# JiehongLin/SAM-6D

Hardware: NVIDIA H100
Metric: poses/sec (higher is better)
Workload: dtype bf16

## Files before the change

include/sam6d_b200.h:

```cpp
#ifndef SAM6D_B200_H
#define SAM6D_B200_H

#ifdef __cplusplus
extern "C" {
#endif


int sam6d_fps(const float* xyz, int b, int n, int m, float* temp, int* idx, void* stream);
int sam6d_fps_single_cta(const float* xyz, int b, int n, int m, float* temp, int* idx, void* stream);

int sam6d_gather_points(const float* points, const int* idx, int b, int c, int n, int m, float* out, void* stream);

int sam6d_gather_rows(const float* src, const int* idx, int b, int n, int m, int c, long long src_bstride, float* out,
                      void* stream);
int sam6d_gather_rows_bf16_f32(const void* src, const int* idx, int b, int n, int m, int c, long long src_bstride, float* out,
                               void* stream);

int sam6d_ball_query(const float* new_xyz, const float* xyz, int b, int n, int m, float radius, int nsample, int* idx,
                     int* cnt, void* stream);
int sam6d_ball_query_pair(const float* new_xyz, const float* xyz, int b, int n, int m, float radius_a, int nsample_a,
                          float radius_b, int nsample_b, int* idx_a, int* idx_b, int* cnt_a, int* cnt_b, void* stream);

int sam6d_group_points(const float* points, const int* idx, int b, int c, int n, int np, int ns, float* out, void* stream);


int sam6d_gemm_f32(const float* A, const float* W, const float* bias, const float* R, float* C, int M, int N, int K,
                   long long lda, long long ldw, long long ldc, long long ldr, int batch, long long sA, long long sW,
                   long long sC, long long sR, float alpha, int relu, void* stream);

int sam6d_gemm_bf16(const void* A, int a_dtype, const void* W, int w_dtype, const float* bias, const float* R, void* C,
                    int c_dtype, int M, int N, int K, long long lda, long long ldw, long long ldc, long long ldr, int batch,
                    long long sA, long long sW, long long sC, long long sR, float alpha, int relu, void* stream);

int sam6d_gemm_tma(const void* A, const void* W, const float* bias, const void* R, void* C, int c_dtype, int M, int N, int K,
                   long long lda, long long ldw, long long ldc, long long ldr, float alpha, int act, void* stream);
int sam6d_gemm_tma_batched(const void* A, const void* W, const float* bias, const void* R, void* C, int c_dtype, int M, int N, int K,
                           long long lda, long long ldw, long long ldc, long long ldr, int batch, long long a_rpb, long long w_rpb,
                           long long c_bs, long long r_bs, float alpha, int act, void* stream);
int sam6d_gemm_tma_vt(const void* A, const void* W, const float* bias, void* C, int M, int N, int K, long long lda, long long ldw,
                      long long ldc, void* Vt, int vt_col0, int vt_S, int vt_N1, void* stream);
int sam6d_gemm_tma_vt2(const void* A, const void* W, const float* bias, void* C, int M, int N, int K, long long lda, long long ldw,
                       long long ldc, void* Vt, int vt_col0, int vt_col1, int vt_S, int vt_N1, void* C2, long long ldc2,
                       void* stream);


int sam6d_layernorm(const float* x, long long x_rpb, long long x_bstride, long long x_ld, float* y, long long y_rpb,
                    long long y_bstride, long long y_ld, const float* gamma, const float* beta, long long rows, int C,
                    float eps, void* stream);
int sam6d_layernorm_bf16(const float* x, long long x_rpb, long long x_bstride, long long x_ld, void* y, long long y_rpb,
                         long long y_bstride, long long y_ld, const float* gamma, const float* beta, long long rows, int C,
                         float eps, void* stream);
int sam6d_layernorm_bf16io(const void* x, long long x_rpb, long long x_bstride, long long x_ld, void* y, long long y_rpb,
                           long long y_bstride, long long y_ld, const float* gamma, const float* beta, long long rows, int C,
                           float eps, void* stream);
int sam6d_l2norm_rows(const float* x, long long x_rpb, long long x_bstride, long long x_ld, float* y, long long y_rpb,
                      long long y_bstride, long long y_ld, long long rows, int C, void* stream);
int sam6d_l2norm_rows_bf16(const float* x, long long x_rpb, long long x_bstride, long long x_ld, void* y, long long y_rpb,
                           long long y_bstride, long long y_ld, long long rows, int C, void* stream);
int sam6d_focus_rows(const float* x, long long x_rpb, long long x_bstride, long long x_ld, float* y, long long y_rpb,
                     long long y_bstride, long long y_ld, const float* softplus_scale, long long rows, int C, void* stream);
int sam6d_rigid_warp(const float* p, const float* R, const float* t, int b, int n, float* out, void* stream);
int sam6d_cloud_radius(const float* po, int b, int n, float* radius, void* stream);
int sam6d_scale_by_radius(const float* src, const float* radius, int b, long long per_batch, float* dst, void* stream);


int sam6d_geo_indices(const float* pts, int b, int S, float sigma_d, float factor_a, float* T, void* stream);
int sam6d_geo_embed_f32(const float* T, long long npairs, const float* div_term, const float* WaT, const float* WdT,
                        const float* bias, float* E, void* stream);

int sam6d_geo_embed_tc(const float* T, long long npairs, const float* div_term, const void* Wa_bf16, const void* Wd_bf16,
                       const float* bias, void* E, int e_is_bf16, void* stream);
int sam6d_geo_embed_dist_tc(const float* T, long long npairs, const float* div_term, const void* Wd_bf16, const float* bias, void* E,
                            void* stream);
int sam6d_geo_embed_lut(const float* T, long long clouds, int S, const void* tabA, int na, float inv_ha, const void* tabD, int nd,
                        float inv_hd, const void* far, const float* div_term, const void* WdT_bf16, const float* bias, void* E,
                        void* stream);


int sam6d_inputs_stage_a(const int* rle_cum, const int* rle_off, int P, int H, int W, const float* depth, double fx, double fy,
                         double cx, double cy, double thr, unsigned char* mask, int* stats, int cap, int* choose1, int* choose2,
                         float* cloud2, void* stream);
int sam6d_inputs_stage_b(const int* stats, const int* keep, int Q, int H, int W, int cap, const int* choose2, const float* cloud2,
                         const int* choose_idx, int ns, int S, const unsigned char* image, const unsigned char* mask, int mask_flag,
                         float* pts, long long* rgb_choose, float* rgb, unsigned char* rgb_u8, void* stream);

int sam6d_crop_resize_normalize(const unsigned char* images, const unsigned char* masks, const int* bbox, int Q, int H, int W, int S,
                                int mask_flag, float* rgb, unsigned char* rgb_u8, void* stream);


int sam6d_crop_resize_pad(const unsigned char* image, const float* masks, const int* boxes, int P, int H, int W, int T, float* rgb,
                          float* pmask, void* stream);
int sam6d_masked_patch_normalize(const float* tokens, long long tok_ld, long long tok_bs, const float* pmask, int P, int G, int patch,
                                 int C, float thresh, float* out_f32, void* out_bf16, unsigned char* valid, void* stream);
int sam6d_appearance_reduce(const float* sim, long long sim_ld, long long sim_bs, int P, int N, const unsigned char* qvalid, float thred,
                            float* appe, float* vis, void* stream);


int sam6d_query_translation(const float* masks, const int* depth, int N, int H, int W, const double* K, double depth_scale,
                            float* translate, void* stream);
int sam6d_project_template_iou(const float* poses, int T, const float* pointcloud, int O, int npc, const long long* best_pose,
                               const long long* pred_obj, const float* translate, const double* K, int N, int H, int W,
                               const long long* boxes, int* image_vu, int* xyxy, float* iou, unsigned char* ok, void* stream);


int sam6d_mask_rle_count(const float* masks, int n, int H, int W, int* col_cnt, int* band_off, int* rle_off, void* stream);
int sam6d_mask_rle_write(const float* masks, int n, int H, int W, const int* col_cnt, const int* band_off, const int* rle_off,
                         int* rle_cum, void* stream);


int sam6d_sam_pe_encode(const float* coords, const float* G, int rows, float* out, void* stream);
int sam6d_sam_mask_embed(const float* masks, const float* params, int B, float* out, void* stream);
int sam6d_sam_self_attn(const float* q, const float* k, const float* v, int B, int T, float* out, void* stream);
int sam6d_sam_tok2img_attn(const float* Q, const void* K, const void* V, long long kv_bs, int B, int T, int L, float* out, void* stream);
int sam6d_sam_img2tok_attn(const void* Q, long long q_bs, const float* Kt, const float* Vt, int B, int T, int L, void* out, void* stream);
int sam6d_sam_ln2d_gelu(const void* x, const float* gamma, const float* beta, long long rows, void* y, void* stream);
int sam6d_sam_mask_dot(const void* up, const float* hyper, int B, int G, float* masks, void* stream);
int sam6d_sam_mask_dot_range(const void* up, const float* hyper, int B, int G, int m0, int nm, float* masks, void* stream);
int sam6d_sam_mask_stats(const float* low, int N, int S, int big, int in_h, int in_w, int H, int W, float thr, float off, int* stats,
                         void* stream);
int sam6d_sam_mask_binarize(const float* low, const int* sel, int K, int S, int big, int in_h, int in_w, int H, int W, float thr,
                            unsigned char* out, void* stream);
int sam6d_sam_mask_upscale(const float* low, int N, int S, int big, int in_h, int in_w, int H, int W, float* out, void* stream);
int sam6d_sam_nms(const float* boxes, int N, float thr, unsigned char* keep, void* stream);


int sam6d_transformer_tail_bf16(const void* hid, long long ld_hid, const void* x, long long ld_x, const void* Wo, const float* bo,
                                const float* g1, const float* b1, const void* We, const float* be, const void* Ws, const float* bs,
                                const float* g2, const float* b2, void* out, long long ld_out, int M, float eps, void* stream);


int sam6d_rpe_scores(const void* E, int e_is_bf16, const float* U, long long u_ld, int B, int S, float* SP, void* stream);
int sam6d_rpe_scores_tc_ld(const void* E, const void* U, int B, int S, float* SP, int sp_ld, void* stream);
int sam6d_mha(const float* Q, long long q_ld, long long q_bs, const float* K, long long k_ld, long long k_bs, const float* V,
              long long v_ld, long long v_bs, const float* bias, int B, int H, int Sq, int Sk, float scale, float* O,
              long long o_ld, long long o_bs, void* stream);
int sam6d_attn_tc(const void* Q, long long q_ld, int q_col0, const void* K, long long k_ld, int k_col0, const void* Vt,
                  long long vt_ld, int B, int H, int Sq, int Sk, int head_dim, int bias_mode, const float* bias,
                  const void* rel_h, const float* rel_w, int Hs, int Ws, const float* bv, float scale, void* out,
                  int out_is_bf16, long long out_ld, void* stream);
int sam6d_attn_tc_bias_ld(const void* Q, long long q_ld, int q_col0, const void* K, long long k_ld, int k_col0, const void* Vt,
                          long long vt_ld, int B, int H, int Sq, int Sk, int head_dim, const float* bias, long long bias_ld,
                          float scale, void* out, int out_is_bf16, long long out_ld, void* stream);
int sam6d_attn_tc_ex(const void* Q, long long q_ld, int q_col0, const void* K, long long k_ld, int k_col0, const void* Vt,
                     long long vt_ld, int B, int H, int Sq, int Sk, int head_dim, float scale, int k_brows, int k_row0, int v_col0,
                     float* lse, void* out, int out_is_bf16, long long out_ld, void* stream);
int sam6d_attn_merge_key(const void* Q, long long q_ld, int q_col0, const void* K, long long k_ld, int k_col0, int k_brows,
                         int key_row, const void* Vt, long long vt_ld, int key_col, const float* lse, int B, int H, int Sq,
                         float scale, void* out, long long out_ld, void* stream);
int sam6d_transpose_tokens_bf16(const void* src, long long ld, int col0, int C, int nB, int L, int N1, void* out, void* stream);
int sam6d_linattn_kv(const float* Kf, long long k_ld, long long k_bs, const float* V, long long v_ld, long long v_bs, int B,
                     int H, int J, float* KV, float* KS, void* stream);
int sam6d_linattn_apply(const float* Qf, long long q_rpb, long long q_bs, long long q_ld, const float* KV, const float* KS,
                        int B, int H, float* X, long long x_bs, long long x_ld, void* stream);
int sam6d_linattn_kv_pack(const float* Kf, long long k_ld, long long k_bs, const float* V, long long v_ld, long long v_bs, int B,
                          int J, void* blob, float* KS, void* stream);
int sam6d_linattn_tc(const void* Q, long long q_ld, long long q_bs, const void* blob, const float* KS,
                     const float* softplus_scale, int B, int rpb, void* X, long long x_ld, long long x_bs, void* stream);

int sam6d_coarse_assign(const float* A, int B, int S, float* W, float* w1, void* stream);
int sam6d_coarse_sample(const float* W, int B, int L, const float* rand, int nr, int* idx, void* stream);
int sam6d_coarse_hypotheses(const int* idx, const float* pts1, const float* pts2, int B, int n, int n1, float* Rt,
                            float* resid, void* stream);
int sam6d_topk_smallest(const float* v, int B, int n, int k, int* out, void* stream);
int sam6d_coarse_select(const float* Rt, const int* top, int B, int n1, int n2, const float* pts1, const float* w1, int n,
                        const float* model, int nm, float* scores, float* R, float* t, void* stream);


int sam6d_pe_mlp_max(const float* pts, const int* idx, const int* cnt, int B, int N, int ns, const float* W1,
                     const float* B1, const float* W2, const float* B2, const float* W3, const float* B3, float* out,
                     int out_ld, int out_off, void* stream);
int sam6d_pe_mlp_max_tc(const float* pts, const int* idx, int B, int N, int ns, const float* W1, const float* B1,
                        const void* W2_bf16, const float* B2, const void* W3_bf16, const float* B3, void* out, int out_is_bf16,
                        int out_ld, int out_off, void* stream);
int sam6d_fine_assign(const float* A, int B, int S, int ld, float shift, const float* pts2, float* rsum, float* csum, float* cpart,
                      int* cpi, int* lab1, int* lab2, float* wts, float* pred, void* stream);
int sam6d_fine_pass_tc(const void* Fa, const void* Fb, int B, int S, float alpha, float shift, int mode, const float* row_f,
                       const float* col_f, int ld_f, const float* q4, float* out_inv, int* lab, float* wts, float* pred, void* stream);
int sam6d_fine_masked_points(const int* lab2, const float* pts2, int B, int S, int ld, float* q4, void* stream);
int sam6d_weighted_procrustes(const float* src, const float* ref, const float* wts, int B, int N, float weight_thresh,
                              float eps, float* R, float* t, void* stream);
int sam6d_pose_score(const float* pts1, const int* lab1, int B, int N, const float* R, const float* t, const float* model,
                     int nm, float dis_thres, const float* radius, float* score, float* t_scaled, void* stream);

int sam6d_bilinear_gather(const void* up, int up_is_bf16, const long long* choose, int B, int K, int G, int sub, int C, int H, int W,
                          float* out, void* stream);

int sam6d_attn_relpos(const float* qkv, long long tok_ld, int nW, int Hs, int Ws, int nH, int head_dim, const float* rel_h,
                      const float* rel_w, float scale, void* out, int out_is_bf16, long long out_ld, void* stream);

int sam6d_attn_global_tc(const void* qkv, long long ld, const void* Vt, long long vt_ld, const void* rel_blob, int B, int H, int grid,
                         float scale, void* out, int out_is_bf16, long long out_ld, void* stream);
int sam6d_attn_global_tc_ex(const void* qkv, long long ld, const void* Vt, long long vt_ld, const void* rel_blob, int B, int H, int grid,
                            int head_dim, float scale, void* out, int out_is_bf16, long long out_ld, void* stream);

int sam6d_template_score(const float* Qn, const float* Rn, int P, int O, int T, int C, float* sim_out, float* obj_score,
                         int* best_obj, float* best_score, int* best_tmpl, void* stream);


int sam6d_render_meshes(const float* verts, const int* faces, const int* mesh_info, int O, int n_verts, int n_faces,
                        const unsigned char* vcol, const float* uv, const unsigned char* tex, const long long* tex_off,
                        const float* base_color, const float* poses, int T, float fx, float fy, float cx, float cy, int H, int W,
                        float znear, float ambient, int* vrec, unsigned long long* vis, int* big, int big_cap, int* counters,
                        unsigned char* rgb, unsigned char* mask, void* xyz, int* tri, float* depth, void* stream);


int sam6d_conv2d_tc(const void* x, long long ldx, int B, int Hi, int Wi, int Cin, const void* w, int k, int stride, int Cout,
                    const float* bias, int silu, const void* r, long long ldr, long long r_bs, void* y, int y_is_f32, long long ldy,
                    long long y_bs, int Wy, int sy, int sx, int oy, int ox, void* stream);
int sam6d_yolo_stem(const unsigned char* img, int B, int H, int W, const float* w, const float* bias, void* out, void* stream);
int sam6d_yolo_sppf(void* buf, long long ld, int B, int H, int W, int C, void* stream);
int sam6d_yolo_upsample2x(const void* x, long long ldx, int B, int H, int W, int C, void* y, long long ldy, void* stream);
int sam6d_yolo_decode(const float* head, long long ld, long long bs, int B, int h0, int w0, int h1, int w1, int h2, int w2, float conf_thr,
                      float* cand, int* count, void* stream);
int sam6d_yolo_masks(const float* proto, int mh, int mw, const float* rows, long long row_ld, int N, int ih, int iw, float kx, float ky,
                     float* low, unsigned char* out, void* stream);

const char* sam6d_version(void);

#ifdef __cplusplus
}
#endif
#endif
```

sam6d_b200/csrc/epilogue.cuh:

```cuda
#pragma once
#include "tc.cuh"

namespace epi {

template <int ACT>
__device__ __forceinline__ float act_fn(float x) {
  if constexpr (ACT == 1) return fmaxf(x, 0.f);
  if constexpr (ACT == 2) return 0.5f * x * (1.f + erff(x * 0.70710678118654752f));
  return x;
}

template <typename T>
struct ident { using type = T; };
__device__ __forceinline__ float ld_res(const float* p) { return *p; }
__device__ __forceinline__ float ld_res(const __nv_bfloat16* p) { return __bfloat162float(*p); }
__device__ __forceinline__ float2 ld_res2(const float* p) { return *reinterpret_cast<const float2*>(p); }
__device__ __forceinline__ float2 ld_res2(const __nv_bfloat16* p) { return __bfloat1622float2(*reinterpret_cast<const __nv_bfloat162*>(p)); }
__device__ __forceinline__ void st1(float* p, float a) { *p = a; }
__device__ __forceinline__ void st1(__nv_bfloat16* p, float a) { *p = __float2bfloat16(a); }
__device__ __forceinline__ void st2(float* p, float a, float b) { *reinterpret_cast<float2*>(p) = make_float2(a, b); }
__device__ __forceinline__ void st2(__nv_bfloat16* p, float a, float b) { *reinterpret_cast<uint32_t*>(p) = tc::pack_bf16(a, b); }

template <typename OT, int ACT, bool HAS_BIAS, bool HAS_RES, typename RT = float, int N>
__device__ __forceinline__ void store_frag(const float (&d)[N / 2], int w, int lane, int row0, int M, int col0, int N_lim, float alpha,
                                           const float* __restrict__ bias, const typename ident<RT>::type* __restrict__ R, long long ldr,
                                           OT* __restrict__ C, long long ldc, int j_lo = 0, int j_hi = N / 8) {
  const bool pairs = ((ldc & 1) == 0) && (!HAS_RES || (ldr & 1) == 0);
#pragma unroll
  for (int j = 0; j < N / 8; ++j) {
    const int col = col0 + tc::frag_col(4 * j, lane);
    if (j < j_lo || j >= j_hi || col >= N_lim) continue;
    const bool two = col + 1 < N_lim;
    float b0 = 0.f, b1 = 0.f;
    if constexpr (HAS_BIAS) { b0 = __ldg(bias + col); if (two) b1 = __ldg(bias + col + 1); }
#pragma unroll
    for (int h = 0; h < 2; ++h) {
      const int row = row0 + tc::frag_row(2 * h, w, lane);
      if (row >= M) continue;
      float x0 = act_fn<ACT>(fmaf(d[4 * j + 2 * h], alpha, b0)), x1 = act_fn<ACT>(fmaf(d[4 * j + 2 * h + 1], alpha, b1));
      const size_t rc = (size_t)row * ldc + col;
      if (two && pairs) {
        if constexpr (HAS_RES) { const float2 r = ld_res2(R + (size_t)row * ldr + col); x0 += r.x; x1 += r.y; }
        st2(C + rc, x0, x1);
      } else {
        if constexpr (HAS_RES) x0 += ld_res(R + (size_t)row * ldr + col);
        st1(C + rc, x0);
        if (two) {
          if constexpr (HAS_RES) x1 += ld_res(R + (size_t)row * ldr + col + 1);
          st1(C + rc + 1, x1);
        }
      }
    }
  }
}

__device__ __forceinline__ void store_frag_swiglu(const float (&d)[128], int w, int lane, int row0, int M, int col0, int out_col0,
                                                  float alpha, const float* __restrict__ bias, __nv_bfloat16* __restrict__ C,
                                                  long long ldc) {
#pragma unroll
  for (int j = 0; j < 16; ++j) {
    const int c = tc::frag_col(4 * j, lane);
    const float g0 = __ldg(bias + col0 + c), g1 = __ldg(bias + col0 + c + 1);
    const float u0 = __ldg(bias + col0 + 128 + c), u1 = __ldg(bias + col0 + 128 + c + 1);
#pragma unroll
    for (int h = 0; h < 2; ++h) {
      const int row = row0 + tc::frag_row(2 * h, w, lane);
      if (row >= M) continue;
      const float x0 = fmaf(d[4 * j + 2 * h], alpha, g0), x1 = fmaf(d[4 * j + 2 * h + 1], alpha, g1);
      const float y0 = fmaf(d[4 * (j + 16) + 2 * h], alpha, u0), y1 = fmaf(d[4 * (j + 16) + 2 * h + 1], alpha, u1);
      st2(C + (size_t)row * ldc + out_col0 + c, x0 / (1.f + __expf(-x0)) * y0, x1 / (1.f + __expf(-x1)) * y1);
    }
  }
}

#define EPI_DISPATCH(ACT_V, BIAS_P, RES_P, ...)                                              \
  do {                                                                                       \
    const int a__ = (ACT_V);                                                                 \
    const bool b__ = (BIAS_P) != nullptr, r__ = (RES_P) != nullptr;                          \
    if (a__ == 0) {                                                                          \
      if (b__) { if (r__) { __VA_ARGS__(0, true, true); } else { __VA_ARGS__(0, true, false); } } \
      else     { if (r__) { __VA_ARGS__(0, false, true); } else { __VA_ARGS__(0, false, false); } } \
    } else if (a__ == 1) {                                                                   \
      if (b__) { if (r__) { __VA_ARGS__(1, true, true); } else { __VA_ARGS__(1, true, false); } } \
      else     { if (r__) { __VA_ARGS__(1, false, true); } else { __VA_ARGS__(1, false, false); } } \
    } else {                                                                                 \
      if (b__) { if (r__) { __VA_ARGS__(2, true, true); } else { __VA_ARGS__(2, true, false); } } \
      else     { if (r__) { __VA_ARGS__(2, false, true); } else { __VA_ARGS__(2, false, false); } } \
    }                                                                                        \
  } while (0)

}
```

sam6d_b200/csrc/fine_tc.cu:

```cuda
#include "common.cuh"
#include "tc.cuh"

namespace {

constexpr int BM = 128, BN = 256, BK = 64, KB = 4, STAGES = 4;
constexpr int A_KB = BM * BK * 2, B_KB = BN * BK * 2;
constexpr int CONSUMERS = 256, NUM_THREADS = CONSUMERS + 128;
constexpr int SMEM_BYTES = KB * A_KB + STAGES * B_KB + 1024;
constexpr float LOG2E = 1.4426950408889634f;

struct FArgs {
  int B, S, mode, ld_f;
  float a2, s2;
  const float* row_f;
  const float* col_f;
  const float4* q4;
  float* out_inv;
  int* lab;
  float* wts; float* pred;
};

__device__ __forceinline__ float ex2(float x) {
  float y;
  asm("ex2.approx.ftz.f32 %0, %1;" : "=f"(y) : "f"(x));
  return y;
}

template <int MODE>
__global__ void __launch_bounds__(NUM_THREADS, 1) fine_pass_kernel(const __grid_constant__ CUtensorMap tmA, const __grid_constant__ CUtensorMap tmB, FArgs g) {
  extern __shared__ __align__(1024) uint8_t smem_raw[];
  uint8_t* smem = reinterpret_cast<uint8_t*>((reinterpret_cast<uintptr_t>(smem_raw) + 1023) & ~(uintptr_t)1023);
  uint8_t* a_res = smem;
  uint8_t* ring = smem + KB * A_KB;
  __shared__ __align__(8) uint64_t a_full, a_empty, full_bar[STAGES], empty_bar[STAGES];
  __shared__ float sc[2][BN];
  __shared__ __align__(16) float4 sq[2][BN];

  const int tid = threadIdx.x, warp = tid >> 5, lane = tid & 31;
  const int m_tiles = (g.S + BM - 1) / BM, n_tiles = (g.S + BN - 1) / BN;
  const int items = g.B * m_tiles;

  if (tid == 0) {
    tc::mbar_init(&a_full, 1); tc::mbar_init(&a_empty, CONSUMERS / 32);
    for (int s = 0; s < STAGES; ++s) { tc::mbar_init(&full_bar[s], 1); tc::mbar_init(&empty_bar[s], CONSUMERS / 32); }
    tc::mbar_fence_init();
    tc::tma_prefetch_desc(&tmA);
    tc::tma_prefetch_desc(&tmB);
  }
  __syncthreads();

  if (warp >= CONSUMERS / 32) {
    tc::producer_regs();
    if (tid == CONSUMERS) {
      long long gk = 0;
      int it = 0;
      for (int item = blockIdx.x; item < items; item += gridDim.x, ++it) {
        const int b = item / m_tiles, mt = item - b * m_tiles;
        tc::mbar_wait(&a_empty, (uint32_t)((it & 1) ^ 1));
        tc::mbar_arrive_expect_tx(&a_full, KB * A_KB);
        for (int kb = 0; kb < KB; ++kb) tc::tma_load_2d(&tmA, &a_full, a_res + kb * A_KB, kb * BK, b * g.S + mt * BM);
        for (int nt = 0; nt < n_tiles; ++nt)
          for (int kb = 0; kb < KB; ++kb, ++gk) {
            const int s = (int)(gk % STAGES);
            tc::mbar_wait(&empty_bar[s], (uint32_t)(((gk / STAGES) & 1) ^ 1));
            tc::mbar_arrive_expect_tx(&full_bar[s], B_KB);
            tc::tma_load_2d(&tmB, &full_bar[s], ring + s * B_KB, kb * BK, b * g.S + nt * BN);
          }
      }
    }
    return;
  }
  tc::consumer_regs();
  const int wg = warp >> 2, w = warp & 3;
  const uint32_t a_addr = tc::smem_u32(a_res) + wg * (64 * 128);
  long long gk = 0, tcount = 0;
  int it = 0;
  for (int item = blockIdx.x; item < items; item += gridDim.x, ++it) {
    const int b = item / m_tiles, mt = item - b * m_tiles;
    float rf[2] = {0.f, 0.f};
#pragma unroll
    for (int hr = 0; hr < 2; ++hr) {
      const int i = mt * BM + wg * 64 + tc::frag_row(2 * hr, w, lane);
      if (MODE != 0 && i < g.S) rf[hr] = g.row_f[(size_t)b * g.ld_f + i];
    }
    const float* cf = (MODE != 0) ? g.col_f + (size_t)b * g.ld_f : nullptr;
    const float4* q4 = (MODE == 2) ? g.q4 + (size_t)b * g.ld_f : nullptr;
    float sum[2] = {0.f, 0.f}, bv[2] = {-INFINITY, -INFINITY}, ws[2] = {0.f, 0.f}, px[2] = {0.f, 0.f}, py[2] = {0.f, 0.f}, pz[2] = {0.f, 0.f};
    int bi[2] = {0x7fffffff, 0x7fffffff};
    tc::mbar_wait(&a_full, (uint32_t)(it & 1));
    for (int nt = 0; nt < n_tiles; ++nt, ++tcount) {
      const int buf = (int)(tcount & 1);
      if (MODE != 0) {
        const int j = nt * BN + tid;
        sc[buf][tid] = (j < g.S) ? cf[j] : 0.f;
        if (MODE == 2) sq[buf][tid] = (j < g.S) ? q4[j] : make_float4(0.f, 0.f, 0.f, 0.f);
        tc::named_bar(1, CONSUMERS);
      }
      float acc[BN / 2];
      int prev = -1;
      for (int kb = 0; kb < KB; ++kb, ++gk) {
        const int s = (int)(gk % STAGES);
        tc::mbar_wait(&full_bar[s], (uint32_t)((gk / STAGES) & 1));
        const uint32_t b_addr = tc::smem_u32(ring + s * B_KB);
        tc::wg_fence();
#pragma unroll
        for (int k = 0; k < BK / 16; ++k)
          tc::wgmma_bf16<BN>(acc, tc::wg_desc(a_addr + kb * A_KB + k * 32), tc::wg_desc(b_addr + k * 32), (kb | k) ? 1u : 0u);
        tc::wg_commit();
        if (prev >= 0) {
          tc::wg_wait<1>();
          if (lane == 0) tc::mbar_arrive(&empty_bar[prev]);
        }
        prev = s;
      }
      tc::wg_wait<0>();
      if (lane == 0) tc::mbar_arrive(&empty_bar[prev]);
      if (nt == n_tiles - 1 && lane == 0) tc::mbar_arrive(&a_empty);
#pragma unroll
      for (int e = 0; e < BN / 2; ++e) {
        const int hr = (e >> 1) & 1, cl = tc::frag_col(e, lane), j = nt * BN + cl;
        const float ev = (j < g.S) ? ex2(fmaf(acc[e], g.a2, -g.s2)) : 0.f;
        if (MODE == 0) {
          sum[hr] += ev;
        } else {
          const float p = (ev * rf[hr]) * (ev * sc[buf][cl]);
          if (p > bv[hr]) { bv[hr] = p; bi[hr] = j; }
          if (MODE == 2) {
            const float4 q = sq[buf][cl];
            const float pm = p * q.w;
            ws[hr] += pm; px[hr] = fmaf(pm, q.x, px[hr]); py[hr] = fmaf(pm, q.y, py[hr]); pz[hr] = fmaf(pm, q.z, pz[hr]);
          }
        }
      }
    }
#pragma unroll
    for (int hr = 0; hr < 2; ++hr) {
      const int i = mt * BM + wg * 64 + tc::frag_row(2 * hr, w, lane);
      if (MODE == 0) {
        const float t = tc::quad_sum(sum[hr]);
        if ((lane & 3) == 0 && i < g.S) g.out_inv[(size_t)b * g.ld_f + i] = 1.f / t;
      } else {
#pragma unroll
        for (int o = 1; o <= 2; o <<= 1) {
          const float ov = __shfl_xor_sync(0xffffffffu, bv[hr], o);
          const int oi = __shfl_xor_sync(0xffffffffu, bi[hr], o);
          if (ov > bv[hr] || (ov == bv[hr] && oi < bi[hr])) { bv[hr] = ov; bi[hr] = oi; }
        }
        float ww = 0.f, qx = 0.f, qy = 0.f, qz = 0.f;
        if (MODE == 2) { ww = tc::quad_sum(ws[hr]); qx = tc::quad_sum(px[hr]); qy = tc::quad_sum(py[hr]); qz = tc::quad_sum(pz[hr]); }
        if ((lane & 3) == 0 && i < g.S) {
          int lb = bi[hr];
          if (lb == 0x7fffffff) lb = 0;
          g.lab[(size_t)b * g.S + i] = lb;
          if (MODE == 2 && i >= 1) {
            if (lb == 0) { ww = 0.f; qx = 0.f; qy = 0.f; qz = 0.f; }
            const size_t o = (size_t)b * (g.S - 1) + (i - 1);
            const float d = ww + 1e-6f;
            g.wts[o] = ww;
            g.pred[o * 3 + 0] = qx / d; g.pred[o * 3 + 1] = qy / d; g.pred[o * 3 + 2] = qz / d;
          }
        }
      }
    }
  }
}

__global__ void fine_masked_points_kernel(const int* __restrict__ lab2, const float* __restrict__ pts2, int S, int ld, float4* __restrict__ q4) {
  const int b = blockIdx.y, j = blockIdx.x * blockDim.x + threadIdx.x;
  if (j >= ld) return;
  float4 q = make_float4(0.f, 0.f, 0.f, 0.f);
  if (j >= 1 && j < S && lab2[(size_t)b * S + j] > 0) {
    const float* p = pts2 + ((size_t)b * (S - 1) + (j - 1)) * 3;
    q = make_float4(p[0], p[1], p[2], 1.f);
  }
  q4[(size_t)b * ld + j] = q;
}

}

S6_API int sam6d_fine_pass_tc(const void* Fa, const void* Fb, int B, int S, float alpha, float shift, int mode, const float* row_f,
                              const float* col_f, int ld_f, const float* q4, float* out_inv, int* lab, float* wts, float* pred,
                              void* stream) {
  S6_REQUIRE(Fa && Fb && B >= 0 && S >= 2 && mode >= 0 && mode <= 2 && ld_f >= S);
  S6_REQUIRE(((reinterpret_cast<uintptr_t>(Fa) | reinterpret_cast<uintptr_t>(Fb)) & 15) == 0 && (long long)B * S < 2000000000LL);
  if (mode == 0) S6_REQUIRE(out_inv != nullptr);
  if (mode >= 1) S6_REQUIRE(row_f && col_f && lab);
  if (mode == 2) S6_REQUIRE(q4 && wts && pred && (reinterpret_cast<uintptr_t>(q4) & 15) == 0);
  if (B == 0) return 0;
  CUtensorMap tmA, tmB;
  int rc = tc::make_map_2d(&tmA, Fa, (long long)B * S, 256, 256, 64, BM);
  if (rc) return rc;
  rc = tc::make_map_2d(&tmB, Fb, (long long)B * S, 256, 256, 64, BN);
  if (rc) return rc;
  int grid;
  S6_CHECK(s6_persistent_grid(B * s6_cdiv(S, BM), 1, &grid));
  FArgs g{B, S, mode, ld_f, alpha * LOG2E, shift * LOG2E, row_f, col_f, reinterpret_cast<const float4*>(q4), out_inv, lab, wts, pred};
  cudaStream_t st = s6_stream(stream);
#define FINE_LAUNCH(M)                                                                                              \
  do {                                                                                                              \
    S6_CHECK(cudaFuncSetAttribute(fine_pass_kernel<M>, cudaFuncAttributeMaxDynamicSharedMemorySize, SMEM_BYTES));   \
    fine_pass_kernel<M><<<grid, NUM_THREADS, SMEM_BYTES, st>>>(tmA, tmB, g);                                        \
  } while (0)
  if (mode == 0) FINE_LAUNCH(0); else if (mode == 1) FINE_LAUNCH(1); else FINE_LAUNCH(2);
#undef FINE_LAUNCH
  S6_LAUNCH_CHECK();
  return 0;
}

S6_API int sam6d_fine_masked_points(const int* lab2, const float* pts2, int B, int S, int ld, float* q4, void* stream) {
  S6_REQUIRE(lab2 && pts2 && q4 && B >= 0 && S >= 2 && ld >= S && (reinterpret_cast<uintptr_t>(q4) & 15) == 0);
  if (B == 0) return 0;
  dim3 grid(s6_cdiv(ld, 256), B);
  fine_masked_points_kernel<<<grid, 256, 0, s6_stream(stream)>>>(lab2, pts2, S, ld, reinterpret_cast<float4*>(q4));
  S6_LAUNCH_CHECK();
  return 0;
}
```

sam6d_b200/csrc/gemm_tma.cu:

```cuda
#include "epilogue.cuh"
#include "tc.cuh"

namespace {

constexpr int BM = 128, BN = 256, BK = 64, STAGES = 4;
constexpr int A_BYTES = BM * BK * 2, B_BYTES = BN * BK * 2, STAGE_BYTES = A_BYTES + B_BYTES;
constexpr int CONSUMERS = 256, THREADS = CONSUMERS + 128;
constexpr int SMEM = STAGES * STAGE_BYTES + 1024;

struct Args {
  const float* bias; const void* R; void* C;
  int M, N, K;
  long long ldc, ldr;
  float alpha;
  int act;
  int batch;
  long long a_rpb, w_rpb;
  long long c_bs, r_bs;
  void* vt; int vt_col0, vt_S, vt_N1, vt_C;
  int vt_col1; void* c2; long long ldc2;
};

template <typename OT, int ACT, bool HAS_BIAS, bool HAS_RES, bool VT = false>
__global__ void __launch_bounds__(THREADS, 1) gemm_tma_kernel(const __grid_constant__ CUtensorMap tmA,
                                                              const __grid_constant__ CUtensorMap tmW, Args g) {
  extern __shared__ __align__(1024) uint8_t smem_raw[];
  uint8_t* smem = reinterpret_cast<uint8_t*>((reinterpret_cast<uintptr_t>(smem_raw) + 1023) & ~(uintptr_t)1023);
  __shared__ __align__(8) uint64_t full_bar[STAGES], empty_bar[STAGES];

  const int tid = threadIdx.x, warp = tid >> 5, lane = tid & 31;
  const int m_tiles = (g.M + BM - 1) / BM, n_tiles = (g.N + BN - 1) / BN;
  const long long tpb = (long long)m_tiles * n_tiles, ntiles = tpb * g.batch;
  const int nkb = (g.K + BK - 1) / BK;

  if (tid == 0) {
    for (int s = 0; s < STAGES; ++s) { tc::mbar_init(&full_bar[s], 1); tc::mbar_init(&empty_bar[s], CONSUMERS / 32); }
    tc::mbar_fence_init();
    tc::tma_prefetch_desc(&tmA);
    tc::tma_prefetch_desc(&tmW);
  }
  s6_pdl_trigger();
  __syncthreads();
  s6_pdl_wait();

  if (warp >= CONSUMERS / 32) {
    tc::producer_regs();
    if (tid == CONSUMERS) {
      long long gk = 0;
      for (long long tile = blockIdx.x; tile < ntiles; tile += gridDim.x) {
        const long long bz = tile / tpb, t = tile - bz * tpb;
        const int m0 = (int)(t % m_tiles) * BM, n0 = (int)(t / m_tiles) * BN;
        const int a_row = (int)(bz * g.a_rpb) + m0, w_row = (int)(bz * g.w_rpb) + n0;
        for (int kb = 0; kb < nkb; ++kb, ++gk) {
          const int s = (int)(gk % STAGES);
          tc::mbar_wait(&empty_bar[s], (uint32_t)(((gk / STAGES) & 1) ^ 1));
          tc::mbar_arrive_expect_tx(&full_bar[s], STAGE_BYTES);
          uint8_t* a_slab = smem + s * STAGE_BYTES;
          tc::tma_load_2d(&tmA, &full_bar[s], a_slab, kb * BK, a_row);
          tc::tma_load_2d(&tmW, &full_bar[s], a_slab + A_BYTES, kb * BK, w_row);
        }
      }
    }
    return;
  }
  tc::consumer_regs();
  const int wg = warp >> 2, w = warp & 3;
  float acc[BN / 2];
  long long gk = 0;
  for (long long tile = blockIdx.x; tile < ntiles; tile += gridDim.x) {
    const long long bz = tile / tpb, t = tile - bz * tpb;
    const int m0 = (int)(t % m_tiles) * BM, n0 = (int)(t / m_tiles) * BN;
    int prev = -1;
    for (int kb = 0; kb < nkb; ++kb, ++gk) {
      const int s = (int)(gk % STAGES);
      tc::mbar_wait(&full_bar[s], (uint32_t)((gk / STAGES) & 1));
      const uint32_t a_addr = tc::smem_u32(smem + s * STAGE_BYTES) + wg * (64 * 128), b_addr = tc::smem_u32(smem + s * STAGE_BYTES) + A_BYTES;
      tc::wg_fence();
#pragma unroll
      for (int k = 0; k < BK / 16; ++k) tc::wgmma_bf16<BN>(acc, tc::wg_desc(a_addr + k * 32), tc::wg_desc(b_addr + k * 32), (kb | k) ? 1u : 0u);
      tc::wg_commit();
      if (prev >= 0) {
        tc::wg_wait<1>();
        if (lane == 0) tc::mbar_arrive(&empty_bar[prev]);
      }
      prev = s;
    }
    tc::wg_wait<0>();
    if (lane == 0) tc::mbar_arrive(&empty_bar[prev]);

    const int row0 = m0 + wg * 64;
    OT* Cb = reinterpret_cast<OT*>(g.C) + bz * g.c_bs;
    const OT* Rb = reinterpret_cast<const OT*>(g.R) + bz * g.r_bs;
    if constexpr (VT) {
      const int jv = min(max((g.vt_col0 - n0) / 8, 0), BN / 8), ju = min(max((g.vt_col1 - n0) / 8, 0), BN / 8);
      epi::store_frag<OT, ACT, HAS_BIAS, false, OT, BN>(acc, w, lane, row0, g.M, n0, g.N, g.alpha, g.bias, nullptr, 0, Cb, g.ldc, 0, jv);
      epi::store_frag<OT, ACT, HAS_BIAS, false, OT, BN>(acc, w, lane, row0, g.M, n0 - g.vt_col1, g.N - g.vt_col1, g.alpha,
                                                        g.bias ? g.bias + g.vt_col1 : nullptr, nullptr, 0, reinterpret_cast<OT*>(g.c2),
                                                        g.ldc2, ju, BN / 8);
#pragma unroll
      for (int j = 0; j < BN / 8; ++j) {
        if (j < jv || j >= ju) continue;
#pragma unroll
        for (int h = 0; h < 2; ++h) {
          const int row = row0 + tc::frag_row(2 * h, w, lane);
          if (row >= g.M) continue;
          const int cloud = row / g.vt_S, tok = row - cloud * g.vt_S;
#pragma unroll
          for (int e = 0; e < 2; ++e) {
            const int col = n0 + tc::frag_col(4 * j + e, lane);
            float x = acc[4 * j + 2 * h + e] * g.alpha;
            if constexpr (HAS_BIAS) x += __ldg(g.bias + col);
            reinterpret_cast<__nv_bfloat16*>(g.vt)[((size_t)cloud * g.vt_C + (col - g.vt_col0)) * g.vt_N1 + tok] =
                __float2bfloat16(epi::act_fn<ACT>(x));
          }
        }
      }
    } else if constexpr (ACT == 3) {
      epi::store_frag_swiglu(acc, w, lane, row0, g.M, n0, n0 / 2, g.alpha, g.bias, Cb, g.ldc);
    } else {
      epi::store_frag<OT, ACT, HAS_BIAS, HAS_RES, OT, BN>(acc, w, lane, row0, g.M, n0, g.N, g.alpha, g.bias, Rb, g.ldr, Cb, g.ldc);
    }
  }
}

int launch_gemm_tma(const void* A, const void* W, const float* bias, const void* R, void* C, int c_dtype, int M, int N, int K,
                    long long lda, long long ldw, long long ldc, long long ldr, int batch, long long a_rpb, long long w_rpb,
                    long long c_bs, long long r_bs, float alpha, int act, void* stream, void* vt = nullptr, int vt_col0 = 0, int vt_S = 1,
                    int vt_N1 = 0, int vt_col1 = -1, void* c2 = nullptr, long long ldc2 = 0) {
  S6_REQUIRE(A && W && C && M >= 0 && N > 0 && K > 0 && (K % 8) == 0 && (lda % 8) == 0 && (ldw % 8) == 0 && act >= 0 && act <= 3);
  S6_REQUIRE((reinterpret_cast<uintptr_t>(A) & 15) == 0 && (reinterpret_cast<uintptr_t>(W) & 15) == 0 && batch >= 0);
  S6_REQUIRE(a_rpb * (long long)batch < 2000000000LL && w_rpb * (long long)batch < 2000000000LL);
  if (M == 0 || batch == 0) return 0;
  CUtensorMap tmA, tmW;
  const long long a_rows = batch > 1 ? a_rpb * (batch - 1) + M : M, w_rows = batch > 1 ? w_rpb * (batch - 1) + N : N;
  int rc = tc::make_map_2d(&tmA, A, a_rows, K, lda, 64, BM);
  if (rc) return rc;
  rc = tc::make_map_2d(&tmW, W, w_rows, K, ldw, 64, BN);
  if (rc) return rc;
  const long long ntiles = (long long)s6_cdiv(M, BM) * s6_cdiv(N, BN) * batch;
  int grid;
  S6_CHECK(s6_persistent_grid(ntiles, 1, &grid));
  if (vt_col1 < 0) vt_col1 = N;
  Args g{bias, R, C, M, N, K, ldc, ldr, alpha, act, batch, a_rpb, w_rpb, c_bs, r_bs, vt, vt_col0, vt_S, vt_N1, vt_col1 - vt_col0,
         vt_col1, c2, ldc2};
  cudaStream_t st = s6_stream(stream);
#define LAUNCH_ONE(OT, ACT, HB, HR, VTK)                                                                               \
  do {                                                                                                                 \
    auto k = gemm_tma_kernel<OT, ACT, HB, HR, VTK>;                                                                    \
    S6_CHECK(cudaFuncSetAttribute(k, cudaFuncAttributeMaxDynamicSharedMemorySize, SMEM));                              \
    S6_CHECK(s6_launch_pdl(k, dim3(grid), dim3(THREADS), SMEM, st, tmA, tmW, g));                                      \
  } while (0)
#define LAUNCH_TMA(ACT, HB, HR)                                                                                        \
  do {                                                                                                                 \
    if (c_dtype) LAUNCH_ONE(__nv_bfloat16, ACT, HB, HR, false); else LAUNCH_ONE(float, ACT, HB, HR, false);           \
  } while (0)
  if (vt) {
    S6_REQUIRE(c_dtype == 1 && bias && !R && act == 0 && batch == 1 && vt_col0 > 0 && vt_col0 < N && (vt_col0 % 32) == 0 && vt_S > 0 &&
               vt_N1 >= vt_S);
    S6_REQUIRE(vt_col1 > vt_col0 && vt_col1 <= N && (vt_col1 % 32) == 0 &&
               (vt_col1 == N || (c2 && (ldc2 % 8) == 0 && ldc2 >= N - vt_col1 && (reinterpret_cast<uintptr_t>(c2) & 15) == 0)));
    LAUNCH_ONE(__nv_bfloat16, 0, true, false, true);
    S6_LAUNCH_CHECK();
    return 0;
  }
  if (act == 3) {
    S6_REQUIRE(c_dtype == 1 && bias && !R && (N % BN) == 0 && (ldc % 2) == 0 && ldc >= N / 2);
    LAUNCH_ONE(__nv_bfloat16, 3, true, false, false);
    S6_LAUNCH_CHECK();
    return 0;
  }
  EPI_DISPATCH(act, bias, R, LAUNCH_TMA);
#undef LAUNCH_TMA
#undef LAUNCH_ONE
  S6_LAUNCH_CHECK();
  return 0;
}

}

S6_API int sam6d_gemm_tma(const void* A, const void* W, const float* bias, const void* R, void* C, int c_dtype, int M, int N, int K,
                          long long lda, long long ldw, long long ldc, long long ldr, float alpha, int act, void* stream) {
  return launch_gemm_tma(A, W, bias, R, C, c_dtype, M, N, K, lda, ldw, ldc, ldr, 1, 0, 0, 0, 0, alpha, act, stream);
}

S6_API int sam6d_gemm_tma_batched(const void* A, const void* W, const float* bias, const void* R, void* C, int c_dtype, int M, int N,
                                  int K, long long lda, long long ldw, long long ldc, long long ldr, int batch, long long a_rpb,
                                  long long w_rpb, long long c_bs, long long r_bs, float alpha, int act, void* stream) {
  S6_REQUIRE(a_rpb >= M && (w_rpb >= N || w_rpb == 0));
  return launch_gemm_tma(A, W, bias, R, C, c_dtype, M, N, K, lda, ldw, ldc, ldr, batch, a_rpb, w_rpb, c_bs, r_bs, alpha, act, stream);
}

S6_API int sam6d_gemm_tma_vt(const void* A, const void* W, const float* bias, void* C, int M, int N, int K, long long lda, long long ldw,
                             long long ldc, void* Vt, int vt_col0, int vt_S, int vt_N1, void* stream) {
  S6_REQUIRE(Vt != nullptr);
  return launch_gemm_tma(A, W, bias, nullptr, C, 1, M, N, K, lda, ldw, ldc, 0, 1, 0, 0, 0, 0, 1.f, 0, stream, Vt, vt_col0, vt_S, vt_N1);
}

S6_API int sam6d_gemm_tma_vt2(const void* A, const void* W, const float* bias, void* C, int M, int N, int K, long long lda, long long ldw,
                              long long ldc, void* Vt, int vt_col0, int vt_col1, int vt_S, int vt_N1, void* C2, long long ldc2,
                              void* stream) {
  S6_REQUIRE(Vt != nullptr && C2 != nullptr);
  return launch_gemm_tma(A, W, bias, nullptr, C, 1, M, N, K, lda, ldw, ldc, 0, 1, 0, 0, 0, 0, 1.f, 0, stream, Vt, vt_col0, vt_S, vt_N1, vt_col1,
                         C2, ldc2);
}
```

sam6d_b200/csrc/tc.cuh:

```cuda
#pragma once
#include <cuda.h>

#include "common.cuh"

namespace tc {

__device__ __forceinline__ uint32_t smem_u32(const void* p) { return (uint32_t)__cvta_generic_to_shared(p); }

__device__ __forceinline__ void mbar_init(uint64_t* bar, uint32_t count) {
  asm volatile("mbarrier.init.shared::cta.b64 [%0], %1;" ::"r"(smem_u32(bar)), "r"(count) : "memory");
}
__device__ __forceinline__ void mbar_fence_init() {
  asm volatile("fence.mbarrier_init.release.cluster;" ::: "memory");
}
__device__ __forceinline__ void mbar_arrive(uint64_t* bar) {
  asm volatile("{\n\t.reg .b64 st;\n\tmbarrier.arrive.shared::cta.b64 st, [%0];\n\t}" ::"r"(smem_u32(bar)) : "memory");
}
__device__ __forceinline__ void mbar_arrive_expect_tx(uint64_t* bar, uint32_t bytes) {
  asm volatile("{\n\t.reg .b64 st;\n\tmbarrier.arrive.expect_tx.shared::cta.b64 st, [%0], %1;\n\t}" ::"r"(smem_u32(bar)), "r"(bytes)
               : "memory");
}
__device__ __forceinline__ bool mbar_try_wait(uint64_t* bar, uint32_t parity) {
  uint32_t ok;
  asm volatile(
      "{\n\t"
      ".reg .pred p;\n\t"
      "mbarrier.try_wait.parity.shared::cta.b64 p, [%1], %2, %3;\n\t"
      "selp.u32 %0, 1, 0, p;\n\t"
      "}"
      : "=r"(ok)
      : "r"(smem_u32(bar)), "r"(parity), "r"(0x989680u)
      : "memory");
  return ok != 0;
}
__device__ __forceinline__ void mbar_wait(uint64_t* bar, uint32_t parity) {
  while (!mbar_try_wait(bar, parity)) {
  }
}

__device__ __forceinline__ void fence_proxy_async_smem() { asm volatile("fence.proxy.async.shared::cta;" ::: "memory"); }

__device__ __forceinline__ uint64_t wg_desc(uint32_t smem_addr) {
  uint64_t d = 0;
  d |= (uint64_t)((smem_addr & 0x3FFFF) >> 4);
  d |= (uint64_t)1 << 16;
  d |= (uint64_t)(1024 >> 4) << 32;
  d |= (uint64_t)1 << 62;
  return d;
}
__device__ __forceinline__ void wg_fence() { asm volatile("wgmma.fence.sync.aligned;" ::: "memory"); }
__device__ __forceinline__ void wg_commit() { asm volatile("wgmma.commit_group.sync.aligned;" ::: "memory"); }
template <int N>
__device__ __forceinline__ void wg_wait() { asm volatile("wgmma.wait_group.sync.aligned %0;" ::"n"(N) : "memory"); }

template <int N>
struct Wgmma;
#define S6_R0 "%0, %1, %2, %3, %4, %5, %6, %7"
#define S6_R1 "%8, %9, %10, %11, %12, %13, %14, %15"
#define S6_R2 "%16, %17, %18, %19, %20, %21, %22, %23"
#define S6_R3 "%24, %25, %26, %27, %28, %29, %30, %31"
#define S6_R4 "%32, %33, %34, %35, %36, %37, %38, %39"
#define S6_R5 "%40, %41, %42, %43, %44, %45, %46, %47"
#define S6_R6 "%48, %49, %50, %51, %52, %53, %54, %55"
#define S6_R7 "%56, %57, %58, %59, %60, %61, %62, %63"
#define S6_R8 "%64, %65, %66, %67, %68, %69, %70, %71"
#define S6_R9 "%72, %73, %74, %75, %76, %77, %78, %79"
#define S6_R10 "%80, %81, %82, %83, %84, %85, %86, %87"
#define S6_R11 "%88, %89, %90, %91, %92, %93, %94, %95"
#define S6_R12 "%96, %97, %98, %99, %100, %101, %102, %103"
#define S6_R13 "%104, %105, %106, %107, %108, %109, %110, %111"
#define S6_R14 "%112, %113, %114, %115, %116, %117, %118, %119"
#define S6_R15 "%120, %121, %122, %123, %124, %125, %126, %127"
#define S6_F4(i) "+f"(d[i]), "+f"(d[i + 1]), "+f"(d[i + 2]), "+f"(d[i + 3])
#define S6_F8(i) S6_F4(i), S6_F4(i + 4)
#define S6_F16(i) S6_F8(i), S6_F8(i + 8)
#define S6_F32(i) S6_F16(i), S6_F16(i + 16)
#define S6_F64(i) S6_F32(i), S6_F32(i + 32)
#define S6_WGMMA(N, REGS, DA, DB, ACC, ...)                                                                                     \
  template <>                                                                                                                \
  struct Wgmma<N> {                                                                                                          \
    __device__ __forceinline__ static void mma(float (&d)[N / 2], uint64_t da, uint64_t db, uint32_t acc) {                 \
      asm volatile("{\n\t.reg .pred p;\n\tsetp.ne.b32 p, " ACC ", 0;\n\twgmma.mma_async.sync.aligned.m64n" #N "k16.f32.bf16.bf16 {" \
                   REGS "}, " DA ", " DB ", p, 1, 1, 0, 0;\n\t}"                                                             \
                   : __VA_ARGS__                                                                                             \
                   : "l"(da), "l"(db), "r"(acc));                                                                            \
    }                                                                                                                        \
  };
S6_WGMMA(16, S6_R0, "%8", "%9", "%10", S6_F8(0))
S6_WGMMA(32, S6_R0 ", " S6_R1, "%16", "%17", "%18", S6_F16(0))
S6_WGMMA(64, S6_R0 ", " S6_R1 ", " S6_R2 ", " S6_R3, "%32", "%33", "%34", S6_F32(0))
S6_WGMMA(80, S6_R0 ", " S6_R1 ", " S6_R2 ", " S6_R3 ", " S6_R4, "%40", "%41", "%42", S6_F32(0), S6_F8(32))
S6_WGMMA(128, S6_R0 ", " S6_R1 ", " S6_R2 ", " S6_R3 ", " S6_R4 ", " S6_R5 ", " S6_R6 ", " S6_R7, "%64", "%65", "%66", S6_F64(0))
S6_WGMMA(256, S6_R0 ", " S6_R1 ", " S6_R2 ", " S6_R3 ", " S6_R4 ", " S6_R5 ", " S6_R6 ", " S6_R7 ", " S6_R8 ", " S6_R9 ", " S6_R10
         ", " S6_R11 ", " S6_R12 ", " S6_R13 ", " S6_R14 ", " S6_R15, "%128", "%129", "%130", S6_F64(0), S6_F64(64))

template <int N>
__device__ __forceinline__ void wgmma_bf16(float (&d)[N / 2], uint64_t da, uint64_t db, uint32_t accumulate) {
  Wgmma<N>::mma(d, da, db, accumulate);
}

__host__ __device__ constexpr int frag_row(int i, int w, int l) { return 16 * w + (l >> 2) + 8 * ((i >> 1) & 1); }
__host__ __device__ constexpr int frag_col(int i, int l) { return 8 * (i >> 2) + 2 * (l & 3) + (i & 1); }

__device__ __forceinline__ float quad_sum(float v) {
  v += __shfl_xor_sync(0xffffffffu, v, 1);
  return v + __shfl_xor_sync(0xffffffffu, v, 2);
}
__device__ __forceinline__ float quad_max(float v) {
  v = fmaxf(v, __shfl_xor_sync(0xffffffffu, v, 1));
  return fmaxf(v, __shfl_xor_sync(0xffffffffu, v, 2));
}

constexpr int kProducerRegs = 40, kConsumerRegs = 232;
__device__ __forceinline__ void producer_regs() { asm volatile("setmaxnreg.dec.sync.aligned.u32 %0;" ::"n"(kProducerRegs)); }
__device__ __forceinline__ void consumer_regs() { asm volatile("setmaxnreg.inc.sync.aligned.u32 %0;" ::"n"(kConsumerRegs)); }

__device__ __forceinline__ void named_bar(int id, int count) { asm volatile("bar.sync %0, %1;" ::"r"(id), "r"(count) : "memory"); }

__device__ __forceinline__ uint32_t sw128_offset(int row, int col) {
  return (uint32_t)(row * 128 + ((((col >> 3) ^ (row & 7)) << 4) | ((col & 7) << 1)));
}

__device__ __forceinline__ void tma_load_2d(const void* tmap, uint64_t* bar, void* smem_dst, int crd0, int crd1) {
  asm volatile("cp.async.bulk.tensor.2d.shared::cluster.global.mbarrier::complete_tx::bytes [%0], [%1, {%3, %4}], [%2];" ::"r"(
                   smem_u32(smem_dst)),
               "l"(reinterpret_cast<uint64_t>(tmap)), "r"(smem_u32(bar)), "r"(crd0), "r"(crd1)
               : "memory");
}
__device__ __forceinline__ void tma_load_3d(const void* tmap, uint64_t* bar, void* smem_dst, int c0, int c1, int c2) {
  asm volatile("cp.async.bulk.tensor.3d.shared::cluster.global.mbarrier::complete_tx::bytes [%0], [%1, {%3, %4, %5}], [%2];" ::"r"(
                   smem_u32(smem_dst)),
               "l"(reinterpret_cast<uint64_t>(tmap)), "r"(smem_u32(bar)), "r"(c0), "r"(c1), "r"(c2)
               : "memory");
}
__device__ __forceinline__ void tma_load_4d(const void* tmap, uint64_t* bar, void* smem_dst, int c0, int c1, int c2, int c3) {
  asm volatile("cp.async.bulk.tensor.4d.shared::cluster.global.mbarrier::complete_tx::bytes [%0], [%1, {%3, %4, %5, %6}], [%2];" ::"r"(
                   smem_u32(smem_dst)),
               "l"(reinterpret_cast<uint64_t>(tmap)), "r"(smem_u32(bar)), "r"(c0), "r"(c1), "r"(c2), "r"(c3)
               : "memory");
}
__device__ __forceinline__ void bulk_load_1d(void* smem_dst, const void* gmem_src, uint32_t bytes, uint64_t* bar) {
  asm volatile("cp.async.bulk.shared::cluster.global.mbarrier::complete_tx::bytes [%0], [%1], %2, [%3];" ::"r"(smem_u32(smem_dst)),
               "l"(reinterpret_cast<uint64_t>(gmem_src)), "r"(bytes), "r"(smem_u32(bar))
               : "memory");
}
__device__ __forceinline__ void tma_prefetch_desc(const void* tmap) {
  asm volatile("prefetch.tensormap [%0];" ::"l"(reinterpret_cast<uint64_t>(tmap)) : "memory");
}

typedef CUresult (*EncodeFn)(CUtensorMap*, CUtensorMapDataType, cuuint32_t, void*, const cuuint64_t*, const cuuint64_t*,
                             const cuuint32_t*, const cuuint32_t*, CUtensorMapInterleave, CUtensorMapSwizzle,
                             CUtensorMapL2promotion, CUtensorMapFloatOOBfill);

inline EncodeFn get_encode() {
  static EncodeFn fn = nullptr;
  if (!fn) {
    void* p = nullptr;
    cudaDriverEntryPointQueryResult q;
    if (cudaGetDriverEntryPoint("cuTensorMapEncodeTiled", &p, cudaEnableDefault, &q) != cudaSuccess || q != cudaDriverEntryPointSuccess)
      return nullptr;
    fn = reinterpret_cast<EncodeFn>(p);
  }
  return fn;
}

inline int encode_map(CUtensorMap* map, const void* ptr, int rank, const cuuint64_t* dims, const cuuint64_t* strides_bytes,
                      const cuuint32_t* box, const cuuint32_t* estr) {
  EncodeFn enc = get_encode();
  if (!enc) return 999;
  CUresult r = enc(map, CU_TENSOR_MAP_DATA_TYPE_BFLOAT16, rank, const_cast<void*>(ptr), dims, strides_bytes, box, estr,
                   CU_TENSOR_MAP_INTERLEAVE_NONE, CU_TENSOR_MAP_SWIZZLE_128B, CU_TENSOR_MAP_L2_PROMOTION_L2_256B,
                   CU_TENSOR_MAP_FLOAT_OOB_FILL_NONE);
  return r == CUDA_SUCCESS ? 0 : 1000 + (int)r;
}

inline int make_map_2d(CUtensorMap* map, const void* ptr, long long rows, long long cols, long long ld, int box_cols, int box_rows) {
  cuuint64_t gdim[2] = {(cuuint64_t)cols, (cuuint64_t)rows};
  cuuint64_t gstride[1] = {(cuuint64_t)ld * 2};
  cuuint32_t box[2] = {(cuuint32_t)box_cols, (cuuint32_t)box_rows};
  cuuint32_t estr[2] = {1, 1};
  return encode_map(map, ptr, 2, gdim, gstride, box, estr);
}

__device__ __forceinline__ bool elect_one() {
  uint32_t pred = 0;
  asm volatile(
      "{\n\t"
      ".reg .pred P;\n\t"
      "elect.sync _|P, 0xffffffff;\n\t"
      "selp.u32 %0, 1, 0, P;\n\t"
      "}"
      : "=r"(pred));
  return pred != 0;
}

__device__ __forceinline__ uint32_t pack_bf16(float a, float b) {
  __nv_bfloat162 h = __floats2bfloat162_rn(a, b);
  return *reinterpret_cast<uint32_t*>(&h);
}

}
```

sam6d_b200/ops.py:

```python
import ctypes
from typing import Optional, Tuple

import torch

from . import _lib

Tensor = torch.Tensor


def _check(t: Tensor, dtype, name: str, ndim: Optional[int] = None):
    if not isinstance(t, torch.Tensor):
        raise RuntimeError(f"{name} must be a torch.Tensor")
    if not t.is_cuda:
        raise RuntimeError(f"{name} must be a CUDA tensor (CPU not supported)")
    if t.dtype != dtype:
        raise RuntimeError(f"{name} must be {dtype}, got {t.dtype}")
    if not t.is_contiguous():
        raise RuntimeError(f"{name} must be contiguous")
    if ndim is not None and t.dim() != ndim:
        raise RuntimeError(f"{name} must have {ndim} dims, got {t.dim()}")


def _p(t: Optional[Tensor]):
    return ctypes.c_void_p(0 if t is None else t.data_ptr())


def _s():
    return ctypes.c_void_p(torch.cuda.current_stream().cuda_stream)


def _ll(v):
    return ctypes.c_longlong(int(v))


def _f(v):
    return ctypes.c_float(float(v))


def furthest_point_sampling(xyz: Tensor, m: int) -> Tensor:
    _check(xyz, torch.float32, "points", 3)
    b, n, c = xyz.shape
    if c != 3:
        raise RuntimeError("points must be (B,N,3)")
    idx = torch.zeros(b, m, dtype=torch.int32, device=xyz.device)
    temp = torch.empty(b, n, dtype=torch.float32, device=xyz.device) if n > 4096 else None
    _lib.call("sam6d_fps", _p(xyz), b, n, int(m), _p(temp), _p(idx), _s())
    return idx


def furthest_point_sampling_single_cta(xyz: Tensor, m: int) -> Tensor:
    _check(xyz, torch.float32, "points", 3)
    b, n, _ = xyz.shape
    idx = torch.zeros(b, m, dtype=torch.int32, device=xyz.device)
    temp = torch.empty(b, n, dtype=torch.float32, device=xyz.device)
    _lib.call("sam6d_fps_single_cta", _p(xyz), b, n, int(m), _p(temp), _p(idx), _s())
    return idx


def gather_points(points: Tensor, idx: Tensor) -> Tensor:
    _check(points, torch.float32, "points", 3)
    _check(idx, torch.int32, "idx", 2)
    b, c, n = points.shape
    m = idx.shape[1]
    out = torch.zeros(b, c, m, dtype=torch.float32, device=points.device)
    _lib.call("sam6d_gather_points", _p(points), _p(idx), b, c, n, m, _p(out), _s())
    return out


def gather_rows(src: Tensor, idx: Tensor, n_rows: Optional[int] = None) -> Tensor:
    _check(src, torch.float32, "src", 3)
    _check(idx, torch.int32, "idx", 2)
    b, n, c = src.shape
    m = idx.shape[1]
    out = torch.empty(b, m, c, dtype=torch.float32, device=src.device)
    _lib.call("sam6d_gather_rows", _p(src), _p(idx), b, n, m, c, _ll(n * c), _p(out), _s())
    return out


def ball_query(new_xyz: Tensor, xyz: Tensor, radius: float, nsample: int, return_count: bool = False):
    _check(new_xyz, torch.float32, "new_xyz", 3)
    _check(xyz, torch.float32, "xyz", 3)
    b, m, _ = new_xyz.shape
    n = xyz.shape[1]
    idx = torch.zeros(b, m, nsample, dtype=torch.int32, device=xyz.device)
    cnt = torch.zeros(b, m, dtype=torch.int32, device=xyz.device) if return_count else None
    _lib.call("sam6d_ball_query", _p(new_xyz), _p(xyz), b, n, m, _f(radius), int(nsample), _p(idx), _p(cnt), _s())
    return (idx, cnt) if return_count else idx


def ball_query_pair(new_xyz: Tensor, xyz: Tensor, ra: float, nsa: int, rb: float, nsb: int):
    _check(new_xyz, torch.float32, "new_xyz", 3)
    _check(xyz, torch.float32, "xyz", 3)
    b, m, _ = new_xyz.shape
    n = xyz.shape[1]
    dev = xyz.device
    ia = torch.empty(b, m, nsa, dtype=torch.int32, device=dev)
    ib = torch.empty(b, m, nsb, dtype=torch.int32, device=dev)
    ca = torch.empty(b, m, dtype=torch.int32, device=dev)
    cb = torch.empty(b, m, dtype=torch.int32, device=dev)
    _lib.call("sam6d_ball_query_pair", _p(new_xyz), _p(xyz), b, n, m, _f(ra), int(nsa), _f(rb), int(nsb), _p(ia), _p(ib), _p(ca),
              _p(cb), _s())
    return ia, ca, ib, cb


def group_points(points: Tensor, idx: Tensor) -> Tensor:
    _check(points, torch.float32, "points", 3)
    _check(idx, torch.int32, "idx", 3)
    b, c, n = points.shape
    _, npnt, ns = idx.shape
    out = torch.zeros(b, c, npnt, ns, dtype=torch.float32, device=points.device)
    _lib.call("sam6d_group_points", _p(points), _p(idx), b, c, n, npnt, ns, _p(out), _s())
    return out


def gemm(A: Tensor, W: Tensor, bias: Optional[Tensor] = None, residual: Optional[Tensor] = None,
         out: Optional[Tensor] = None, relu=False, alpha: float = 1.0) -> Tensor:
    _check(A, torch.float32, "A", 2)
    _check(W, torch.float32, "W", 2)
    M, K = A.shape
    N = W.shape[0]
    if W.shape[1] != K:
        raise RuntimeError("gemm: inner dimensions differ")
    if out is None:
        out = torch.empty(M, N, dtype=torch.float32, device=A.device)
    _lib.call("sam6d_gemm_f32", _p(A), _p(W), _p(bias), _p(residual), _p(out), M, N, K, _ll(K), _ll(K), _ll(N), _ll(N),
              1, _ll(0), _ll(0), _ll(0), _ll(0), _f(alpha), int(relu), _s())
    return out


def gemm_raw(A_ptr, W_ptr, bias, R_ptr, C_ptr, M, N, K, lda, ldw, ldc, ldr, batch=1, sA=0, sW=0, sC=0, sR=0,
             alpha=1.0, relu=False):
    _lib.call("sam6d_gemm_f32", ctypes.c_void_p(A_ptr), ctypes.c_void_p(W_ptr), _p(bias), ctypes.c_void_p(R_ptr or 0),
              ctypes.c_void_p(C_ptr), int(M), int(N), int(K), _ll(lda), _ll(ldw), _ll(ldc), _ll(ldr), int(batch), _ll(sA),
              _ll(sW), _ll(sC), _ll(sR), _f(alpha), int(relu), _s())


_DT = {torch.float32: 0, torch.bfloat16: 1}


def gemm_tc_raw(A_ptr, a_dt, W_ptr, w_dt, bias, R_ptr, C_ptr, c_dt, M, N, K, lda, ldw, ldc, ldr, batch=1, sA=0, sW=0, sC=0, sR=0,
                alpha=1.0, relu=False):
    _lib.call("sam6d_gemm_bf16", ctypes.c_void_p(A_ptr), int(a_dt), ctypes.c_void_p(W_ptr), int(w_dt), _p(bias),
              ctypes.c_void_p(R_ptr or 0), ctypes.c_void_p(C_ptr), int(c_dt), int(M), int(N), int(K), _ll(lda), _ll(ldw), _ll(ldc),
              _ll(ldr), int(batch), _ll(sA), _ll(sW), _ll(sC), _ll(sR), _f(alpha), int(relu), _s())


def gemm_tc(A: Tensor, W: Tensor, bias: Optional[Tensor] = None, residual: Optional[Tensor] = None, out: Optional[Tensor] = None,
            relu: bool = False, alpha: float = 1.0, out_dtype=torch.float32) -> Tensor:
    for t, n in ((A, "A"), (W, "W")):
        if t.dtype not in _DT:
            raise RuntimeError(f"{n} must be float32 or bfloat16")
        _check(t, t.dtype, n, 2)
    M, K = A.shape
    N = W.shape[0]
    if W.shape[1] != K:
        raise RuntimeError("gemm: inner dimensions differ")
    if out is None:
        out = torch.empty(M, N, dtype=out_dtype, device=A.device)
    gemm_tc_raw(A.data_ptr(), _DT[A.dtype], W.data_ptr(), _DT[W.dtype], bias, residual.data_ptr() if residual is not None else 0,
                out.data_ptr(), _DT[out.dtype], M, N, K, K, K, N, N, alpha=alpha, relu=relu)
    return out


def gemm_tma(A: Tensor, W: Tensor, bias: Optional[Tensor] = None, residual: Optional[Tensor] = None, out: Optional[Tensor] = None,
             act: int = 0, alpha: float = 1.0, out_dtype=torch.float32) -> Tensor:
    _check(A, torch.bfloat16, "A", 2)
    _check(W, torch.bfloat16, "W", 2)
    M, K = A.shape
    N = W.shape[0]
    if W.shape[1] != K:
        raise RuntimeError("gemm: inner dimensions differ")
    Nout = N // 2 if act == ACT_SWIGLU else N
    if out is None:
        out = torch.empty(M, Nout, dtype=torch.bfloat16 if act == ACT_SWIGLU else out_dtype, device=A.device)
    if residual is not None:
        _check(residual, out.dtype, "residual", 2)
    _lib.call("sam6d_gemm_tma", _p(A), _p(W), _p(bias), _p(residual), _p(out), _DT[out.dtype], M, N, K, _ll(K), _ll(K), _ll(Nout), _ll(N),
              _f(alpha), int(act), _s())
    return out


ACT_SWIGLU = 3


def pack_swiglu_rows(t: Tensor, block: int = 128) -> Tensor:
    H = t.shape[0] // 2
    if t.shape[0] != 2 * H or H % block:
        raise ValueError(f"SwiGLU w12 needs 2H rows with H % {block} == 0, got {t.shape[0]}")
    rest = t.shape[1:]
    return t.reshape(2, H // block, block, *rest).transpose(0, 1).reshape(2 * H, *rest).contiguous()


_VT_CACHE = {}


def _vt_buffer(rows: int, n1: int, device, slot: int) -> Tensor:
    key = (rows, n1, str(device), slot, torch.cuda.current_stream(device).cuda_stream)
    buf = _VT_CACHE.get(key)
    if buf is None:
        if len(_VT_CACHE) > 64:
            _VT_CACHE.clear()
        buf = torch.zeros(rows, n1, dtype=torch.bfloat16, device=device)
        _VT_CACHE[key] = buf
    return buf


def gemm_tma_vt(A: Tensor, W: Tensor, bias: Tensor, vt_col0: int, S: int, slot: int = 0) -> Tuple[Tensor, Tensor]:
    _check(A, torch.bfloat16, "A", 2)
    _check(W, torch.bfloat16, "W", 2)
    M, K = A.shape
    N = W.shape[0]
    if W.shape[1] != K or M % S or not (0 < vt_col0 < N):
        raise RuntimeError("gemm_tma_vt: shape mismatch")
    n1 = (S + 15) // 16 * 16
    out = torch.empty(M, vt_col0, dtype=torch.bfloat16, device=A.device)
    vt = _vt_buffer((M // S) * (N - vt_col0), n1, A.device, slot)
    _lib.call("sam6d_gemm_tma_vt", _p(A), _p(W), _p(bias), _p(out), M, N, K, _ll(K), _ll(K), _ll(vt_col0), _p(vt), int(vt_col0), int(S),
              int(n1), _s())
    return out, vt


def gemm_tma_vt2(A: Tensor, W: Tensor, bias: Tensor, vt_col0: int, vt_col1: int, S: int, slot: int = 0) -> Tuple[Tensor, Tensor, Tensor]:
    _check(A, torch.bfloat16, "A", 2)
    _check(W, torch.bfloat16, "W", 2)
    M, K = A.shape
    N = W.shape[0]
    if W.shape[1] != K or M % S or not (0 < vt_col0 < vt_col1 < N):
        raise RuntimeError("gemm_tma_vt2: shape mismatch")
    n1 = (S + 15) // 16 * 16
    out = torch.empty(M, vt_col0, dtype=torch.bfloat16, device=A.device)
    out2 = torch.empty(M, N - vt_col1, dtype=torch.bfloat16, device=A.device)
    vt = _vt_buffer((M // S) * (vt_col1 - vt_col0), n1, A.device, slot)
    _lib.call("sam6d_gemm_tma_vt2", _p(A), _p(W), _p(bias), _p(out), M, N, K, _ll(K), _ll(K), _ll(vt_col0), _p(vt), int(vt_col0),
              int(vt_col1), int(S), int(n1), _p(out2), _ll(N - vt_col1), _s())
    return out, vt, out2


def layernorm_raw(x_ptr, x_view, y_ptr, y_view, gamma: Tensor, beta: Tensor, rows: int, C: int, eps: float = 1e-5):
    _lib.call("sam6d_layernorm", ctypes.c_void_p(x_ptr), _ll(x_view[0]), _ll(x_view[1]), _ll(x_view[2]),
              ctypes.c_void_p(y_ptr), _ll(y_view[0]), _ll(y_view[1]), _ll(y_view[2]), _p(gamma), _p(beta), _ll(rows), int(C),
              _f(eps), _s())


def layernorm(x: Tensor, gamma: Tensor, beta: Tensor, eps: float = 1e-5, out: Optional[Tensor] = None) -> Tensor:
    _check(x, torch.float32, "x")
    C = x.shape[-1]
    rows = x.numel() // C
    if out is None:
        out = torch.empty_like(x)
    layernorm_raw(x.data_ptr(), (rows, 0, C), out.data_ptr(), (rows, 0, C), gamma, beta, rows, C, eps)
    return out


def layernorm_bf16(x: Tensor, gamma: Tensor, beta: Tensor, eps: float = 1e-5) -> Tensor:
    _check(x, torch.float32, "x")
    C = x.shape[-1]
    rows = x.numel() // C
    out = torch.empty(x.shape, dtype=torch.bfloat16, device=x.device)
    _lib.call("sam6d_layernorm_bf16", _p(x), _ll(rows), _ll(0), _ll(C), _p(out), _ll(rows), _ll(0), _ll(C), _p(gamma), _p(beta),
              _ll(rows), int(C), _f(eps), _s())
    return out


def layernorm_bf16io(x: Tensor, gamma: Tensor, beta: Tensor, eps: float = 1e-5, out: Optional[Tensor] = None) -> Tensor:
    _check(x, torch.bfloat16, "x")
    C = x.shape[-1]
    rows = x.numel() // C
    if out is None:
        out = torch.empty_like(x)
    _lib.call("sam6d_layernorm_bf16io", _p(x), _ll(max(rows, 1)), _ll(0), _ll(C), _p(out), _ll(max(rows, 1)), _ll(0), _ll(C),
              _p(gamma), _p(beta), _ll(rows), int(C), _f(eps), _s())
    return out


def transformer_tail_bf16(hid: Tensor, x: Tensor, wo: Tensor, bo: Tensor, g1: Tensor, b1: Tensor, we: Tensor, be: Tensor, ws: Tensor,
                          bs: Tensor, g2: Tensor, b2: Tensor, out: Optional[Tensor] = None, eps: float = 1e-5) -> Tensor:
    _check(hid, torch.bfloat16, "hid", 2)
    _check(x, torch.bfloat16, "x", 2)
    M = hid.shape[0]
    if hid.shape[1] != 256 or x.shape != hid.shape or wo.shape != (256, 256) or we.shape != (512, 256) or ws.shape != (256, 512):
        raise RuntimeError("transformer_tail_bf16: d_model 256, hidden 512")
    for w in (wo, we, ws):
        _check(w, torch.bfloat16, "weight", 2)
    if out is None:
        out = torch.empty_like(hid)
    _check(out, torch.bfloat16, "out", 2)
    _lib.call("sam6d_transformer_tail_bf16", _p(hid), _ll(256), _p(x), _ll(256), _p(wo), _p(bo), _p(g1), _p(b1), _p(we), _p(be), _p(ws),
              _p(bs), _p(g2), _p(b2), _p(out), _ll(256), int(M), _f(eps), _s())
    return out


def gather_rows_bf16_f32(src: Tensor, idx: Tensor) -> Tensor:
    _check(src, torch.bfloat16, "src", 3)
    _check(idx, torch.int32, "idx", 2)
    b, n, c = src.shape
    m = idx.shape[1]
    out = torch.empty(b, m, c, dtype=torch.float32, device=src.device)
    _lib.call("sam6d_gather_rows_bf16_f32", _p(src), _p(idx), b, n, m, c, _ll(n * c), _p(out), _s())
    return out


def gather_rows_bf16(src: Tensor, idx: Tensor) -> Tensor:
    _check(src, torch.bfloat16, "src", 3)
    _check(idx, torch.int32, "idx", 2)
    b, n, c = src.shape
    m = idx.shape[1]
    out = torch.empty(b, m, c, dtype=torch.bfloat16, device=src.device)
    _lib.call("sam6d_gather_rows", _p(src), _p(idx), b, n, m, c // 2, _ll(n * c // 2), _p(out), _s())
    return out


def l2norm_rows(x: Tensor) -> Tensor:
    _check(x, torch.float32, "x")
    C = x.shape[-1]
    rows = x.numel() // C
    out = torch.empty_like(x)
    _lib.call("sam6d_l2norm_rows", _p(x), _ll(rows), _ll(0), _ll(C), _p(out), _ll(rows), _ll(0), _ll(C), _ll(rows), C, _s())
    return out


def l2norm_rows_bf16(x: Tensor) -> Tensor:
    _check(x, torch.float32, "x")
    C = x.shape[-1]
    rows = x.numel() // C
    out = torch.empty(x.shape, dtype=torch.bfloat16, device=x.device)
    _lib.call("sam6d_l2norm_rows_bf16", _p(x), _ll(max(rows, 1)), _ll(0), _ll(C), _p(out), _ll(max(rows, 1)), _ll(0), _ll(C), _ll(rows), C,
              _s())
    return out


def gemm_tma_batched(A: Tensor, W: Tensor, out: Tensor, M: int, N: int, ldc: int, c_bs: int, alpha: float = 1.0,
                     bias: Optional[Tensor] = None, residual: Optional[Tensor] = None, ldr: int = 0, r_bs: int = 0) -> Tensor:
    _check(A, torch.bfloat16, "A", 3)
    _check(W, torch.bfloat16, "W")
    batch, a_rows, K = A.shape
    shared = W.dim() == 2
    if W.shape[-1] != K or a_rows < M or (not shared and (W.shape[0] != batch or W.shape[1] < N)) or (shared and W.shape[0] != N):
        raise RuntimeError("gemm_tma_batched: shape mismatch")
    if residual is not None and residual.dtype != out.dtype:
        raise RuntimeError("gemm_tma_batched: the residual must have the output's element type")
    _lib.call("sam6d_gemm_tma_batched", _p(A), _p(W), _p(bias), _p(residual), _p(out), _DT[out.dtype], int(M), int(N), int(K), _ll(K),
              _ll(K), _ll(ldc), _ll(ldr), int(batch), _ll(a_rows), _ll(0 if shared else W.shape[1]), _ll(c_bs), _ll(r_bs), _f(alpha), 0,
              _s())
    return out


def focus_rows_raw(x_ptr, x_view, y_ptr, y_view, sp_scale: Tensor, rows: int, C: int):
    _lib.call("sam6d_focus_rows", ctypes.c_void_p(x_ptr), _ll(x_view[0]), _ll(x_view[1]), _ll(x_view[2]),
              ctypes.c_void_p(y_ptr), _ll(y_view[0]), _ll(y_view[1]), _ll(y_view[2]), _p(sp_scale), _ll(rows), int(C), _s())


def rigid_warp(p: Tensor, R: Tensor, t: Tensor) -> Tensor:
    _check(p, torch.float32, "p", 3)
    _check(R, torch.float32, "R", 3)
    _check(t, torch.float32, "t", 2)
    out = torch.empty_like(p)
    _lib.call("sam6d_rigid_warp", _p(p), _p(R), _p(t), p.shape[0], p.shape[1], _p(out), _s())
    return out


def cloud_radius(po: Tensor) -> Tensor:
    _check(po, torch.float32, "dense_po", 3)
    r = torch.empty(po.shape[0], dtype=torch.float32, device=po.device)
    _lib.call("sam6d_cloud_radius", _p(po), po.shape[0], po.shape[1], _p(r), _s())
    return r


def scale_by_radius(x: Tensor, radius: Tensor) -> Tensor:
    _check(x, torch.float32, "x")
    _check(radius, torch.float32, "radius", 1)
    out = torch.empty_like(x)
    b = x.shape[0]
    _lib.call("sam6d_scale_by_radius", _p(x), _p(radius), b, _ll(x.numel() // max(b, 1)), _p(out), _s())
    return out


def geo_indices(pts: Tensor, sigma_d: float, factor_a: float) -> Tensor:
    _check(pts, torch.float32, "points", 3)
    b, s, _ = pts.shape
    T = torch.empty(b, s, s, 4, dtype=torch.float32, device=pts.device)
    _lib.call("sam6d_geo_indices", _p(pts), b, s, _f(sigma_d), _f(factor_a), _p(T), _s())
    return T


def geo_embed_f32(T: Tensor, div_term: Tensor, WaT: Tensor, WdT: Tensor, bias: Tensor) -> Tensor:
    _check(T, torch.float32, "T", 4)
    b, s, _, _ = T.shape
    E = torch.empty(b, s, s, 256, dtype=torch.float32, device=T.device)
    _lib.call("sam6d_geo_embed_f32", _p(T), _ll(b * s * s), _p(div_term), _p(WaT), _p(WdT), _p(bias), _p(E), _s())
    return E


def geo_embed_tc(T: Tensor, div_term: Tensor, Wa_bf16: Tensor, Wd_bf16: Tensor, bias: Tensor, out_dtype=torch.bfloat16) -> Tensor:
    _check(T, torch.float32, "T", 4)
    _check(Wa_bf16, torch.bfloat16, "Wa", 2)
    _check(Wd_bf16, torch.bfloat16, "Wd", 2)
    b, s, _, _ = T.shape
    E = torch.empty(b, s, s, 256, dtype=out_dtype, device=T.device)
    _lib.call("sam6d_geo_embed_tc", _p(T), _ll(b * s * s), _p(div_term), _p(Wa_bf16), _p(Wd_bf16), _p(bias), _p(E),
              int(out_dtype == torch.bfloat16), _s())
    return E


def geo_embed_dist_tc(T: Tensor, div_term: Tensor, Wd_bf16: Tensor, bias: Tensor) -> Tensor:
    if T.dtype != torch.float32 or not T.is_cuda or not T.is_contiguous() or T.shape[-1] != 4:
        raise RuntimeError("T must be a contiguous CUDA float32 tensor (..., 4)")
    _check(Wd_bf16, torch.bfloat16, "Wd", 2)
    n = T.numel() // 4
    E = torch.empty(*T.shape[:-1], 256, dtype=torch.bfloat16, device=T.device)
    _lib.call("sam6d_geo_embed_dist_tc", _p(T), _ll(n), _p(div_term), _p(Wd_bf16), _p(bias), _p(E), _s())
    return E


def geo_embed_lut(T: Tensor, tabA: Tensor, inv_ha: float, tabD: Tensor, inv_hd: float, far: Tensor, div_term: Tensor, WdT_bf16: Tensor,
                  bias: Tensor) -> Tensor:
    _check(T, torch.float32, "T", 4)
    _check(tabA, torch.bfloat16, "tabA", 2)
    _check(tabD, torch.bfloat16, "tabD", 2)
    _check(far, torch.bfloat16, "far", 4)
    _check(WdT_bf16, torch.bfloat16, "WdT", 2)
    b, s, _, _ = T.shape
    if far.shape != (b, 2, s, 256) or tabA.shape[1] != 256 or tabD.shape[1] != 256 or T.shape[3] != 4:
        raise RuntimeError("geo_embed_lut: shape mismatch")
    E = torch.empty(b, s, s, 256, dtype=torch.bfloat16, device=T.device)
    _lib.call("sam6d_geo_embed_lut", _p(T), _ll(b), s, _p(tabA), tabA.shape[0], _f(inv_ha), _p(tabD), tabD.shape[0], _f(inv_hd), _p(far),
              _p(div_term), _p(WdT_bf16), _p(bias), _p(E), _s())
    return E


def rpe_scores(E: Tensor, U: Tensor, u_ptr: Optional[int] = None, u_ld: int = 1024) -> Tensor:
    if E.dtype not in (torch.float32, torch.bfloat16):
        raise RuntimeError("E must be float32 or bfloat16")
    _check(E, E.dtype, "E", 4)
    if u_ptr is None:
        _check(U, torch.float32, "U", 4)
        u_ptr = U.data_ptr()
    B, S = E.shape[0], E.shape[1]
    SP = torch.empty(B, 4, S, S, dtype=torch.float32, device=E.device)
    _lib.call("sam6d_rpe_scores", _p(E), int(E.dtype == torch.bfloat16), ctypes.c_void_p(u_ptr), _ll(u_ld), B, S, _p(SP), _s())
    return SP


def rpe_scores_tc(E: Tensor, U: Tensor, ld: Optional[int] = None) -> Tensor:
    _check(E, torch.bfloat16, "E", 4)
    _check(U, torch.bfloat16, "U", 2)
    B, S = E.shape[0], E.shape[1]
    if U.shape != (B * S, 1024) or E.shape[3] != 256 or E.shape[2] != S:
        raise RuntimeError("rpe_scores_tc: E (B,S,S,256), U (B*S,1024)")
    ld = S if ld is None else ld
    SP = torch.empty(B, 4, S, ld, dtype=torch.float32, device=E.device)
    _lib.call("sam6d_rpe_scores_tc_ld", _p(E), _p(U), B, S, _p(SP), int(ld), _s())
    return SP


def rpe_scores_tc_padded(E: Tensor, U: Tensor) -> Tensor:
    return rpe_scores_tc(E, U, ld=(E.shape[1] + 15) // 16 * 16)


def attn_tc_padded_bias(Q: Tensor, q_col0: int, K: Tensor, k_col0: int, Vt: Tensor, B: int, H: int, Sq: int, Sk: int, D: int,
                        scale: float, bias: Tensor, out_dtype=torch.bfloat16) -> Tensor:
    _check(Q, torch.bfloat16, "Q", 2)
    _check(K, torch.bfloat16, "K", 2)
    _check(Vt, torch.bfloat16, "Vt", 2)
    _check(bias, torch.float32, "bias", 4)
    if bias.shape[:3] != (B, H, Sq) or bias.shape[3] < Sk or bias.shape[3] % 4:
        raise RuntimeError("attn_tc_padded_bias: bias (B,H,Sq,ld), ld >= Sk, ld % 4 == 0")
    out = torch.empty(B * Sq, H * D, dtype=out_dtype, device=Q.device)
    _lib.call("sam6d_attn_tc_bias_ld", _p(Q), _ll(Q.shape[1]), int(q_col0), _p(K), _ll(K.shape[1]), int(k_col0), _p(Vt), _ll(Vt.shape[1]),
              int(B), int(H), int(Sq), int(Sk), int(D), _p(bias), _ll(bias.shape[3]), _f(scale), _p(out),
              int(out_dtype == torch.bfloat16), _ll(H * D), _s())
    return out


def mha_raw(q_ptr, q_ld, q_bs, k_ptr, k_ld, k_bs, v_ptr, v_ld, v_bs, bias: Optional[Tensor], B, H, Sq, Sk, scale,
            o_ptr, o_ld, o_bs):
    _lib.call("sam6d_mha", ctypes.c_void_p(q_ptr), _ll(q_ld), _ll(q_bs), ctypes.c_void_p(k_ptr), _ll(k_ld), _ll(k_bs),
              ctypes.c_void_p(v_ptr), _ll(v_ld), _ll(v_bs), _p(bias), int(B), int(H), int(Sq), int(Sk), _f(scale),
              ctypes.c_void_p(o_ptr), _ll(o_ld), _ll(o_bs), _s())


def pack_rel_pos(rel_h: Tensor, rel_w: Tensor, slab_rows: int = 32) -> Tensor:
    D = rel_h.shape[1]
    DS = (D + 63) // 64
    if rel_h.shape[0] > slab_rows or rel_w.shape[0] > slab_rows:
        raise RuntimeError("pack_rel_pos: table has more rows than the slab")
    blob = torch.zeros(2 * DS * slab_rows * 64, dtype=torch.bfloat16, device=rel_h.device)
    j = torch.arange(slab_rows, device=rel_h.device).view(slab_rows, 1)
    c = torch.arange(D, device=rel_h.device).view(1, D)
    off = j * 64 + ((((c % 64) // 8) ^ (j % 8)) * 8) + (c % 8)
    for t, tab in enumerate((rel_h, rel_w)):
        n = tab.shape[0]
        idx = ((t * DS + c // 64) * slab_rows * 64 + off)[:n]
        blob[idx.reshape(-1)] = tab.to(torch.bfloat16).reshape(-1)
    return blob


def attn_global_tc(qkv: Tensor, vt: Tensor, rel_blob: Tensor, B: int, H: int, grid: int, scale: float, out_dtype=torch.bfloat16,
                   D: int = 80) -> Tensor:
    _check(qkv, torch.bfloat16, "qkv", 2)
    _check(vt, torch.bfloat16, "vt", 2)
    _check(rel_blob, torch.bfloat16, "rel_blob", 1)
    L = grid * grid
    out = torch.empty(B * L, H * D, dtype=out_dtype, device=qkv.device)
    _lib.call("sam6d_attn_global_tc_ex", _p(qkv), _ll(qkv.shape[1]), _p(vt), _ll(vt.shape[1]), _p(rel_blob), int(B), int(H), int(grid),
              int(D), _f(scale), _p(out), int(out_dtype == torch.bfloat16), _ll(H * D), _s())
    return out


def attn_tc(Q: Tensor, q_col0: int, K: Tensor, k_col0: int, Vt: Tensor, B: int, H: int, Sq: int, Sk: int, D: int, scale: float,
            bias: Optional[Tensor] = None, rel: Optional[tuple] = None, bv: Optional[Tensor] = None,
            out_dtype=torch.float32) -> Tensor:
    _check(Q, torch.bfloat16, "Q", 2)
    _check(K, torch.bfloat16, "K", 2)
    _check(Vt, torch.bfloat16, "Vt", 2)
    mode, rh, rw, Hs, Ws = 0, None, None, 0, 0
    if bias is not None:
        _check(bias, torch.float32, "bias", 4)
        mode = 1
    elif rel is not None:
        rh, Hs, Ws = rel
        mode = 2
    out = torch.empty(B * Sq, H * D, dtype=out_dtype, device=Q.device)
    _lib.call("sam6d_attn_tc", _p(Q), _ll(Q.shape[1]), int(q_col0), _p(K), _ll(K.shape[1]), int(k_col0), _p(Vt), _ll(Vt.shape[1]),
              int(B), int(H), int(Sq), int(Sk), int(D), mode, _p(bias), _p(rh), _p(rw), int(Hs), int(Ws), _p(bv), _f(scale), _p(out),
              int(out_dtype == torch.bfloat16), _ll(H * D), _s())
    return out


def attn_tc_ex(Q: Tensor, q_col0: int, K: Tensor, k_col0: int, Vt: Tensor, B: int, H: int, Sq: int, Sk: int, D: int, scale: float,
               k_brows: int, k_row0: int = 0, v_col0: int = 0, want_lse: bool = False, out_dtype=torch.bfloat16):
    _check(Q, torch.bfloat16, "Q", 2)
    _check(K, torch.bfloat16, "K", 2)
    _check(Vt, torch.bfloat16, "Vt", 2)
    out = torch.empty(B * Sq, H * D, dtype=out_dtype, device=Q.device)
    lse = torch.empty(B, H, Sq, dtype=torch.float32, device=Q.device) if want_lse else None
    _lib.call("sam6d_attn_tc_ex", _p(Q), _ll(Q.shape[1]), int(q_col0), _p(K), _ll(K.shape[1]), int(k_col0), _p(Vt), _ll(Vt.shape[1]),
              int(B), int(H), int(Sq), int(Sk), int(D), _f(scale), int(k_brows), int(k_row0), int(v_col0), _p(lse), _p(out),
              int(out_dtype == torch.bfloat16), _ll(H * D), _s())
    return out, lse


def attn_merge_key(Q: Tensor, q_col0: int, K: Tensor, k_col0: int, k_brows: int, key_row: int, Vt: Tensor, key_col: int, lse: Tensor,
                   B: int, H: int, Sq: int, scale: float, out: Tensor) -> Tensor:
    _check(out, torch.bfloat16, "out", 2)
    _check(lse, torch.float32, "lse", 3)
    _lib.call("sam6d_attn_merge_key", _p(Q), _ll(Q.shape[1]), int(q_col0), _p(K), _ll(K.shape[1]), int(k_col0), int(k_brows), int(key_row),
              _p(Vt), _ll(Vt.shape[1]), int(key_col), _p(lse), int(B), int(H), int(Sq), _f(scale), _p(out), _ll(out.shape[1]), _s())
    return out


def transpose_tokens(src: Tensor, col0: int, C: int, nB: int, L: int) -> Tensor:
    _check(src, torch.bfloat16, "src", 2)
    N1 = (L + 15) // 16 * 16
    out = torch.empty(nB * C, N1, dtype=torch.bfloat16, device=src.device)
    _lib.call("sam6d_transpose_tokens_bf16", _p(src), _ll(src.shape[1]), int(col0), int(C), int(nB), int(L), int(N1), _p(out), _s())
    return out


def linattn_kv_raw(k_ptr, k_ld, k_bs, v_ptr, v_ld, v_bs, B, H, J, KV: Tensor, KS: Tensor):
    _lib.call("sam6d_linattn_kv", ctypes.c_void_p(k_ptr), _ll(k_ld), _ll(k_bs), ctypes.c_void_p(v_ptr), _ll(v_ld), _ll(v_bs),
              int(B), int(H), int(J), _p(KV), _p(KS), _s())


def linattn_apply_raw(q_ptr, q_rpb, q_bs, q_ld, KV: Tensor, KS: Tensor, B, H, x_ptr, x_bs, x_ld):
    _lib.call("sam6d_linattn_apply", ctypes.c_void_p(q_ptr), _ll(q_rpb), _ll(q_bs), _ll(q_ld), _p(KV), _p(KS), int(B), int(H),
              ctypes.c_void_p(x_ptr), _ll(x_bs), _ll(x_ld), _s())


def linattn_kv_pack_raw(k_ptr, k_ld, k_bs, v_ptr, v_ld, v_bs, B, J, device):
    blob = torch.empty(B, 4 * 64 * 64, dtype=torch.bfloat16, device=device)
    KS = torch.empty(B, 4, 64, dtype=torch.float32, device=device)
    _lib.call("sam6d_linattn_kv_pack", ctypes.c_void_p(k_ptr), _ll(k_ld), _ll(k_bs), ctypes.c_void_p(v_ptr), _ll(v_ld), _ll(v_bs),
              int(B), int(J), _p(blob), _p(KS), _s())
    return blob, KS


def linattn_tc_raw(q_ptr, q_ld, q_bs, blob: Tensor, KS: Tensor, sp_scale: Tensor, B, rpb, x_ptr, x_ld, x_bs):
    _lib.call("sam6d_linattn_tc", ctypes.c_void_p(q_ptr), _ll(q_ld), _ll(q_bs), _p(blob), _p(KS), _p(sp_scale), int(B), int(rpb),
              ctypes.c_void_p(x_ptr), _ll(x_ld), _ll(x_bs), _s())


def coarse_assign(A: Tensor) -> Tuple[Tensor, Tensor]:
    _check(A, torch.float32, "atten", 3)
    B, S, _ = A.shape
    n = S - 1
    W = torch.empty(B, n * n, dtype=torch.float32, device=A.device)
    w1 = torch.empty(B, n, dtype=torch.float32, device=A.device)
    _lib.call("sam6d_coarse_assign", _p(A), B, S, _p(W), _p(w1), _s())
    return W, w1


def coarse_sample(W: Tensor, rand: Tensor) -> Tensor:
    _check(W, torch.float32, "W", 2)
    _check(rand, torch.float32, "rand", 2)
    B, L = W.shape
    nr = rand.shape[1]
    idx = torch.empty(B, nr, dtype=torch.int32, device=W.device)
    _lib.call("sam6d_coarse_sample", _p(W), B, L, _p(rand), nr, _p(idx), _s())
    return idx


def coarse_hypotheses(idx: Tensor, pts1: Tensor, pts2: Tensor) -> Tuple[Tensor, Tensor]:
    _check(idx, torch.int32, "idx", 2)
    _check(pts1, torch.float32, "pts1", 3)
    _check(pts2, torch.float32, "pts2", 3)
    B, n, _ = pts1.shape
    n1 = idx.shape[1] // 3
    Rt = torch.empty(B, n1, 12, dtype=torch.float32, device=idx.device)
    resid = torch.empty(B, n1, dtype=torch.float32, device=idx.device)
    _lib.call("sam6d_coarse_hypotheses", _p(idx), _p(pts1), _p(pts2), B, n, n1, _p(Rt), _p(resid), _s())
    return Rt, resid


def topk_smallest(v: Tensor, k: int) -> Tensor:
    _check(v, torch.float32, "v", 2)
    B, n = v.shape
    out = torch.empty(B, k, dtype=torch.int32, device=v.device)
    _lib.call("sam6d_topk_smallest", _p(v), B, n, int(k), _p(out), _s())
    return out


def coarse_select(Rt: Tensor, top: Tensor, pts1: Tensor, w1: Tensor, model: Tensor):
    _check(Rt, torch.float32, "Rt", 3)
    _check(top, torch.int32, "top", 2)
    _check(model, torch.float32, "model", 3)
    B, n1, _ = Rt.shape
    n2 = top.shape[1]
    n = pts1.shape[1]
    scores = torch.empty(B, n2, dtype=torch.float32, device=Rt.device)
    R = torch.empty(B, 3, 3, dtype=torch.float32, device=Rt.device)
    t = torch.empty(B, 3, dtype=torch.float32, device=Rt.device)
    _lib.call("sam6d_coarse_select", _p(Rt), _p(top), B, n1, n2, _p(pts1), _p(w1), n, _p(model), model.shape[1], _p(scores),
              _p(R), _p(t), _s())
    return R, t, scores


def pe_mlp_max(pts: Tensor, idx: Tensor, cnt: Tensor, weights, out: Tensor, out_off: int):
    _check(pts, torch.float32, "pts", 3)
    _check(idx, torch.int32, "idx", 3)
    _check(cnt, torch.int32, "cnt", 2)
    B, N, _ = pts.shape
    ns = idx.shape[2]
    W1, B1, W2, B2, W3, B3 = weights
    _lib.call("sam6d_pe_mlp_max", _p(pts), _p(idx), _p(cnt), B, N, ns, _p(W1), _p(B1), _p(W2), _p(B2), _p(W3), _p(B3),
              _p(out), out.shape[-1], int(out_off), _s())


def pe_mlp_max_tc(pts: Tensor, idx: Tensor, weights, out: Tensor, out_off: int):
    _check(pts, torch.float32, "pts", 3)
    _check(idx, torch.int32, "idx", 3)
    B, N, _ = pts.shape
    ns = idx.shape[2]
    W1, B1, W2, B2, W3, B3 = weights
    _check(W2, torch.bfloat16, "W2", 2)
    _check(W3, torch.bfloat16, "W3", 2)
    if out.dtype not in (torch.float32, torch.bfloat16):
        raise RuntimeError("pe_mlp_max_tc: out must be float32 or bfloat16")
    _lib.call("sam6d_pe_mlp_max_tc", _p(pts), _p(idx), B, N, ns, _p(W1), _p(B1), _p(W2), _p(B2), _p(W3), _p(B3), _p(out),
              int(out.dtype == torch.bfloat16), out.shape[-1], int(out_off), _s())


def fine_assign(A: Tensor, pts2: Tensor, shift: float):
    if A.dim() != 3 or A.dtype != torch.float32 or not A.is_cuda:
        raise RuntimeError("atten must be a CUDA fp32 (B,S,S) tensor")
    _check(pts2, torch.float32, "pts2", 3)
    B, S, _ = A.shape
    if A.stride(2) != 1 or A.stride(0) != S * A.stride(1) or A.stride(1) % 4 or A.data_ptr() % 16:
        ld = (S + 3) // 4 * 4
        store = torch.empty(B, S, ld, dtype=torch.float32, device=A.device)
        store[:, :, :S] = A
        A = store[:, :, :S]
    ld = A.stride(1)
    dev = A.device
    tiles = (S + 31) // 32
    if tiles < 4:
        raise RuntimeError("fine_assign: S >= 97 required")
    rsum = torch.empty(B, ld, dtype=torch.float32, device=dev)
    csum = torch.empty(B, ld, dtype=torch.float32, device=dev)
    cpart = torch.empty(B, tiles, ld, dtype=torch.float32, device=dev)
    cpi = torch.empty(B, tiles, ld, dtype=torch.int32, device=dev)
    lab1 = torch.zeros(B, S, dtype=torch.int32, device=dev)
    lab2 = torch.zeros(B, S, dtype=torch.int32, device=dev)
    wts = torch.empty(B, S - 1, dtype=torch.float32, device=dev)
    pred = torch.empty(B, S - 1, 3, dtype=torch.float32, device=dev)
    _lib.call("sam6d_fine_assign", _p(A), B, S, int(ld), _f(shift), _p(pts2), _p(rsum), _p(csum), _p(cpart), _p(cpi), _p(lab1),
              _p(lab2), _p(wts), _p(pred), _s())
    return lab1, lab2, wts, pred


def fine_assign_tc(f1n: Tensor, f2n: Tensor, pts2: Tensor, alpha: float):
    _check(f1n, torch.bfloat16, "f1n", 3)
    _check(f2n, torch.bfloat16, "f2n", 3)
    _check(pts2, torch.float32, "pts2", 3)
    B, S, C = f1n.shape
    if C != 256 or f2n.shape != f1n.shape or pts2.shape[1] != S - 1:
        raise RuntimeError("fine_assign_tc: (B,S,256) tokens and (B,S-1,3) points expected")
    dev = f1n.device
    ld = (S + 3) // 4 * 4
    rinv = torch.empty(B, ld, dtype=torch.float32, device=dev)
    cinv = torch.empty(B, ld, dtype=torch.float32, device=dev)
    q4 = torch.empty(B, ld, 4, dtype=torch.float32, device=dev)
    lab1 = torch.zeros(B, S, dtype=torch.int32, device=dev)
    lab2 = torch.zeros(B, S, dtype=torch.int32, device=dev)
    wts = torch.empty(B, S - 1, dtype=torch.float32, device=dev)
    pred = torch.empty(B, S - 1, 3, dtype=torch.float32, device=dev)
    a, sh = _f(alpha), _f(alpha)
    _lib.call("sam6d_fine_pass_tc", _p(f1n), _p(f2n), B, S, a, sh, 0, None, None, ld, None, _p(rinv), None, None, None, _s())
    _lib.call("sam6d_fine_pass_tc", _p(f2n), _p(f1n), B, S, a, sh, 0, None, None, ld, None, _p(cinv), None, None, None, _s())
    _lib.call("sam6d_fine_pass_tc", _p(f2n), _p(f1n), B, S, a, sh, 1, _p(cinv), _p(rinv), ld, None, None, _p(lab2), None, None, _s())
    _lib.call("sam6d_fine_masked_points", _p(lab2), _p(pts2), B, S, ld, _p(q4), _s())
    _lib.call("sam6d_fine_pass_tc", _p(f1n), _p(f2n), B, S, a, sh, 2, _p(rinv), _p(cinv), ld, _p(q4), None, _p(lab1), _p(wts), _p(pred),
              _s())
    return lab1, lab2, wts, pred


def weighted_procrustes(src: Tensor, ref: Tensor, wts: Tensor, weight_thresh: float = 0.0, eps: float = 1e-5):
    _check(src, torch.float32, "src", 3)
    _check(ref, torch.float32, "ref", 3)
    _check(wts, torch.float32, "weights", 2)
    B, N, _ = src.shape
    R = torch.empty(B, 3, 3, dtype=torch.float32, device=src.device)
    t = torch.empty(B, 3, dtype=torch.float32, device=src.device)
    _lib.call("sam6d_weighted_procrustes", _p(src), _p(ref), _p(wts), B, N, _f(weight_thresh), _f(eps), _p(R), _p(t), _s())
    return R, t


def pose_score(pts1: Tensor, lab1: Tensor, R: Tensor, t: Tensor, model: Tensor, radius: Tensor, dis_thres: float = 0.15):
    _check(pts1, torch.float32, "pts1", 3)
    _check(lab1, torch.int32, "lab1", 2)
    B, N, _ = pts1.shape
    score = torch.empty(B, dtype=torch.float32, device=pts1.device)
    ts = torch.empty(B, 3, dtype=torch.float32, device=pts1.device)
    _lib.call("sam6d_pose_score", _p(pts1), _p(lab1), B, N, _p(R), _p(t), _p(model), model.shape[1], _f(dis_thres),
              _p(radius), _p(score), _p(ts), _s())
    return score, ts


def attn_relpos(qkv: Tensor, nW: int, Hs: int, Ws: int, nH: int, rel_h: Tensor, rel_w: Tensor, scale: float,
                out_dtype=torch.float32) -> Tensor:
    _check(qkv, torch.float32, "qkv", 2)
    _check(rel_h, torch.float32, "rel_pos_h", 2)
    _check(rel_w, torch.float32, "rel_pos_w", 2)
    T, C3 = qkv.shape
    C = C3 // 3
    if T != nW * Hs * Ws or rel_h.shape[0] != 2 * Hs - 1 or rel_w.shape[0] != 2 * Ws - 1:
        raise RuntimeError("attn_relpos: shape mismatch")
    out = torch.empty(T, C, dtype=out_dtype, device=qkv.device)
    _lib.call("sam6d_attn_relpos", _p(qkv), _ll(C3), int(nW), int(Hs), int(Ws), int(nH), C // nH, _p(rel_h), _p(rel_w), _f(scale),
              _p(out), int(out_dtype == torch.bfloat16), _ll(C), _s())
    return out


def bilinear_gather(up: Tensor, choose: Tensor, G: int, sub: int, C: int, H: int, W: int) -> Tensor:
    if up.dtype not in (torch.float32, torch.bfloat16):
        raise RuntimeError("bilinear_gather: up must be float32 or bfloat16")
    _check(up, up.dtype, "up", 3)
    _check(choose, torch.int64, "choose", 2)
    B, K = choose.shape
    if up.shape != (B, G * G, sub * sub * C):
        raise RuntimeError("bilinear_gather: shape mismatch")
    out = torch.empty(B, K, C, dtype=torch.float32, device=up.device)
    _lib.call("sam6d_bilinear_gather", _p(up), int(up.dtype == torch.bfloat16), _p(choose), int(B), int(K), int(G), int(sub), int(C),
              int(H), int(W), _p(out), _s())
    return out


def template_score(Qn: Tensor, Rn: Tensor, want_sim: bool = True):
    _check(Qn, torch.float32, "query", 2)
    _check(Rn, torch.float32, "reference", 3)
    P, C = Qn.shape
    O, T, _ = Rn.shape
    dev = Qn.device
    sim = torch.empty(P, O, T, dtype=torch.float32, device=dev) if want_sim else None
    obj = torch.empty(P, O, dtype=torch.float32, device=dev)
    bo = torch.zeros(P, dtype=torch.int32, device=dev)
    bs = torch.zeros(P, dtype=torch.float32, device=dev)
    bt = torch.zeros(P, dtype=torch.int32, device=dev)
    _lib.call("sam6d_template_score", _p(Qn), _p(Rn), P, O, T, C, _p(sim), _p(obj), _p(bo), _p(bs), _p(bt), _s())
    return sim, obj, bo, bs, bt


def mask_rle(masks: Tensor) -> Tuple[Tensor, Tensor]:
    _check(masks, torch.float32, "masks", 3)
    n, H, W = masks.shape
    dev = masks.device
    col_cnt = torch.empty(n, W, dtype=torch.int32, device=dev)
    band_off = torch.empty(n, (W + 31) // 32, dtype=torch.int32, device=dev)
    rle_off = torch.empty(n + 1, dtype=torch.int32, device=dev)
    _lib.call("sam6d_mask_rle_count", _p(masks), n, H, W, _p(col_cnt), _p(band_off), _p(rle_off), _s())
    rle_cum = torch.empty(int(rle_off[n]), dtype=torch.int32, device=dev)
    _lib.call("sam6d_mask_rle_write", _p(masks), n, H, W, _p(col_cnt), _p(band_off), _p(rle_off), _p(rle_cum), _s())
    return rle_cum, rle_off
```

sam6d_b200/pem.py:

```python
import math
from types import SimpleNamespace
from typing import Dict, Optional

import torch
import torch.nn as nn

from . import ops

NUM_HEADS = 4

PRECISIONS = ("fp32", "bf16")
RPE_TC = True
PADDED_BIAS = True
GEO_LUT_INV_H = 8.0
GEO_LUT_D_MAX = 32.0


class _W:
    __slots__ = ("f32", "bf16")

    def __init__(self, w: torch.Tensor):
        self.f32 = w.detach().to(torch.float32).contiguous()
        self.bf16 = self.f32.to(torch.bfloat16).contiguous()


def _gemm(prec, A, W: "_W", bias=None, residual=None, relu=False):
    if prec == "bf16":
        if A.dtype == torch.bfloat16 and residual is None and A.is_contiguous() and A.shape[1] % 64 == 0:
            return ops.gemm_tma(A, W.bf16, bias, act=1 if relu else 0)
        return ops.gemm_tc(A, W.bf16, bias, residual=residual, relu=relu)
    return ops.gemm(A, W.f32, bias, residual=residual, relu=relu)


def _gemm_raw(prec, A_ptr, W: "_W", bias, R_ptr, C_ptr, M, N, K, lda, ldc, ldr=0, batch=1, sA=0, sC=0, sR=0):
    if prec == "bf16":
        ops.gemm_tc_raw(A_ptr, 0, W.bf16.data_ptr(), 1, bias, R_ptr, C_ptr, 0, M, N, K, lda, K, ldc, ldr, batch=batch, sA=sA, sW=0,
                        sC=sC, sR=sR)
    else:
        ops.gemm_raw(A_ptr, W.f32.data_ptr(), bias, R_ptr, C_ptr, M, N, K, lda, K, ldc, ldr, batch=batch, sA=sA, sW=0, sC=sC, sR=sR)


def _cfg(cfg, **defaults):
    if isinstance(cfg, dict):
        cfg = SimpleNamespace(**cfg)
    for k, v in defaults.items():
        if not hasattr(cfg, k):
            setattr(cfg, k, v)
    return cfg


class _MHAParams(nn.Module):
    def __init__(self, d_model, rpe: bool):
        super().__init__()
        self.proj_q = nn.Linear(d_model, d_model)
        self.proj_k = nn.Linear(d_model, d_model)
        self.proj_v = nn.Linear(d_model, d_model)
        if rpe:
            self.proj_p = nn.Linear(d_model, d_model)


class _AttentionLayerParams(nn.Module):
    def __init__(self, d_model, rpe: bool):
        super().__init__()
        self.attention = _MHAParams(d_model, rpe)
        self.linear = nn.Linear(d_model, d_model)
        self.norm = nn.LayerNorm(d_model)


class _AttentionOutputParams(nn.Module):
    def __init__(self, d_model):
        super().__init__()
        self.expand = nn.Linear(d_model, d_model * 2)
        self.squeeze = nn.Linear(d_model * 2, d_model)
        self.norm = nn.LayerNorm(d_model)


class _TransformerLayerParams(nn.Module):
    def __init__(self, d_model, rpe: bool):
        super().__init__()
        self.attention = _AttentionLayerParams(d_model, rpe)
        self.output = _AttentionOutputParams(d_model)


class _Packed:

    def __init__(self):
        self.key = None
        self.w = {}


def _param_key(module: nn.Module):
    return tuple((p.data_ptr(), p._version) for p in module.parameters()) + tuple(
        (b.data_ptr(), b._version) for b in module.buffers())


def _f32(t: torch.Tensor) -> torch.Tensor:
    return t.detach().to(torch.float32).contiguous()


def _stack2(a: torch.Tensor, b: torch.Tensor) -> Optional[torch.Tensor]:
    if (a.shape == b.shape and a.dtype == b.dtype and a.is_contiguous() and b.is_contiguous() and a.device == b.device
            and a.untyped_storage().data_ptr() == b.untyped_storage().data_ptr()
            and b.storage_offset() == a.storage_offset() + a.numel()):
        return torch.as_strided(a, (2 * a.shape[0],) + tuple(a.shape[1:]), a.stride(), a.storage_offset())
    return None


def _attn_tail(prec, x2d: torch.Tensor, hid: torch.Tensor, lw) -> torch.Tensor:
    y = _gemm(prec, hid, lw["wo"], lw["bo"], residual=x2d)
    y = ops.layernorm(y, lw["g1"], lw["b1"])
    h = _gemm(prec, y, lw["we"], lw["be"], relu=True)
    z = _gemm(prec, h, lw["ws"], lw["bs"], residual=y)
    return ops.layernorm(z, lw["g2"], lw["b2"])


def _pack_tail(layer: nn.Module) -> Dict[str, torch.Tensor]:
    a, o = layer.attention, layer.output
    return dict(wo=_W(a.linear.weight), bo=_f32(a.linear.bias), g1=_f32(a.norm.weight), b1=_f32(a.norm.bias),
                we=_W(o.expand.weight), be=_f32(o.expand.bias), ws=_W(o.squeeze.weight), bs=_f32(o.squeeze.bias),
                g2=_f32(o.norm.weight), b2=_f32(o.norm.bias))


def _tail_bf16(x2d: torch.Tensor, hid: torch.Tensor, lw, out: Optional[torch.Tensor] = None) -> torch.Tensor:
    return ops.transformer_tail_bf16(hid, x2d, lw["wo"].bf16, lw["bo"], lw["g1"], lw["b1"], lw["we"].bf16, lw["be"],
                                     lw["ws"].bf16, lw["bs"], lw["g2"], lw["b2"], out=out)


class GeometricTransformer(nn.Module):

    def __init__(self, blocks, d_model, num_heads, dropout=None, activation_fn='ReLU', return_attention_scores=False,
                 parallel=False):
        super().__init__()
        if list(blocks) != ['self', 'cross'] or parallel or return_attention_scores or dropout:
            raise ValueError("sam6d_b200.GeometricTransformer supports the configuration SAM-6D uses: "
                             "blocks=['self','cross'], parallel=False, dropout=None, no attention-score output")
        if activation_fn != 'ReLU' or num_heads != NUM_HEADS or d_model != 256:
            raise ValueError("sam6d_b200 kernels are built for d_model=256, num_heads=4, ReLU")
        self.blocks = list(blocks)
        self.d_model, self.num_heads = d_model, num_heads
        self.layers = nn.ModuleList([_TransformerLayerParams(d_model, rpe=True), _TransformerLayerParams(d_model, rpe=False)])
        self._packed = _Packed()
        self.precision = "fp32"

    def _weights(self):
        key = _param_key(self)
        if self._packed.key != key:
            C, H = self.d_model, self.num_heads
            d = C // H
            sa = self.layers[0].attention.attention
            wq, bq = _f32(sa.proj_q.weight), _f32(sa.proj_q.bias)
            wp = _f32(sa.proj_p.weight)
            mu = [wp[h * d:(h + 1) * d, :].t().double() @ wq[h * d:(h + 1) * d, :].double() for h in range(H)]
            cu = [wp[h * d:(h + 1) * d, :].t().double() @ bq[h * d:(h + 1) * d].double() for h in range(H)]
            w_self = torch.cat([wq, _f32(sa.proj_k.weight), _f32(sa.proj_v.weight)] + [m.float() for m in mu], dim=0)
            b_self = torch.cat([bq, _f32(sa.proj_k.bias), _f32(sa.proj_v.bias)] + [c.float() for c in cu], dim=0)
            ca = self.layers[1].attention.attention
            self._packed.w = dict(
                w_self=_W(w_self), b_self=b_self.contiguous(), tail_self=_pack_tail(self.layers[0]),
                w_qkv=_W(w_self[:3 * C]), b_qkv=b_self[:3 * C].contiguous(), w_u=_W(w_self[3 * C:]), b_u=b_self[3 * C:].contiguous(),
                wq_c=_W(ca.proj_q.weight), bq_c=_f32(ca.proj_q.bias),
                wkv_c=_W(torch.cat([_f32(ca.proj_k.weight), _f32(ca.proj_v.weight)], dim=0)),
                bkv_c=torch.cat([_f32(ca.proj_k.bias), _f32(ca.proj_v.bias)], dim=0).contiguous(),
                wkqv_c=_W(torch.cat([_f32(ca.proj_k.weight), _f32(ca.proj_q.weight), _f32(ca.proj_v.weight)], dim=0)),
                bkqv_c=torch.cat([_f32(ca.proj_k.bias), _f32(ca.proj_q.bias), _f32(ca.proj_v.bias)], dim=0).contiguous(),
                tail_cross=_pack_tail(self.layers[1]))
            self._packed.key = key
        return self._packed.w

    def _self_layer(self, x: torch.Tensor, emb: torch.Tensor, w) -> torch.Tensor:
        B, S, C = x.shape
        x2d = x.reshape(B * S, C)
        if self.precision == "bf16" and S <= 256:
            d = C // NUM_HEADS
            qkv = ops.gemm_tc(x2d, w["w_qkv"].bf16, w["b_qkv"], out_dtype=torch.bfloat16)
            u = ops.gemm_tc(x2d, w["w_u"].bf16, w["b_u"])
            sp = ops.rpe_scores(emb, None, u_ptr=u.data_ptr(), u_ld=NUM_HEADS * C)
            vt = ops.transpose_tokens(qkv, 2 * C, C, B, S)
            hid = ops.attn_tc(qkv, 0, qkv, C, vt, B, NUM_HEADS, S, S, d, 1.0 / math.sqrt(d), bias=sp)
            return _attn_tail(self.precision, x2d, hid, w["tail_self"]).view(B, S, C)
        ld = 3 * C + NUM_HEADS * C
        qkvu = _gemm(self.precision, x2d, w["w_self"], w["b_self"])
        base, f = qkvu.data_ptr(), 4
        sp = ops.rpe_scores(emb, None, u_ptr=base + 3 * C * f, u_ld=ld)
        hid = torch.empty(B * S, C, dtype=torch.float32, device=x.device)
        ops.mha_raw(base, ld, S * ld, base + C * f, ld, S * ld, base + 2 * C * f, ld, S * ld, sp, B, NUM_HEADS, S, S,
                    1.0 / math.sqrt(C // NUM_HEADS), hid.data_ptr(), C, S * C)
        return _attn_tail(self.precision, x2d, hid, w["tail_self"]).view(B, S, C)

    def _cross_layer(self, x: torch.Tensor, mem: torch.Tensor, w) -> torch.Tensor:
        B, S, C = x.shape
        Sm = mem.shape[1]
        x2d = x.reshape(B * S, C)
        if self.precision == "bf16" and Sm <= 256:
            d = C // NUM_HEADS
            q = ops.gemm_tc(x2d, w["wq_c"].bf16, w["bq_c"], out_dtype=torch.bfloat16)
            kv = ops.gemm_tc(mem.reshape(B * Sm, C), w["wkv_c"].bf16, w["bkv_c"], out_dtype=torch.bfloat16)
            vt = ops.transpose_tokens(kv, C, C, B, Sm)
            hid = ops.attn_tc(q, 0, kv, 0, vt, B, NUM_HEADS, S, Sm, d, 1.0 / math.sqrt(d))
            return _attn_tail(self.precision, x2d, hid, w["tail_cross"]).view(B, S, C)
        q = _gemm(self.precision, x2d, w["wq_c"], w["bq_c"])
        kv = _gemm(self.precision, mem.reshape(B * Sm, C), w["wkv_c"], w["bkv_c"])
        hid = torch.empty(B * S, C, dtype=torch.float32, device=x.device)
        ops.mha_raw(q.data_ptr(), C, S * C, kv.data_ptr(), 2 * C, Sm * 2 * C, kv.data_ptr() + C * 4, 2 * C, Sm * 2 * C, None,
                    B, NUM_HEADS, S, Sm, 1.0 / math.sqrt(C // NUM_HEADS), hid.data_ptr(), C, S * C)
        return _attn_tail(self.precision, x2d, hid, w["tail_cross"]).view(B, S, C)

    def _self_bf16(self, x, emb, w):
        B, S, C = x.shape
        d = C // NUM_HEADS
        x2d = x.view(B * S, C)
        if S <= 200 and emb.dtype == torch.bfloat16:
            qk, vt, u = ops.gemm_tma_vt2(x2d, w["w_self"].bf16, w["b_self"], 2 * C, 3 * C, S)
            sp = ops.rpe_scores_tc_padded(emb, u)
            hid = ops.attn_tc_padded_bias(qk, 0, qk, C, vt, B, NUM_HEADS, S, S, d, 1.0 / math.sqrt(d), sp)
            return _tail_bf16(x2d, hid, w["tail_self"]).view(B, S, C)
        qk, vt = ops.gemm_tma_vt(x2d, w["w_qkv"].bf16, w["b_qkv"], 2 * C, S)
        u = ops.gemm_tma(x2d, w["w_u"].bf16, w["b_u"])
        sp = ops.rpe_scores(emb, None, u_ptr=u.data_ptr(), u_ld=NUM_HEADS * C)
        hid = ops.attn_tc(qk, 0, qk, C, vt, B, NUM_HEADS, S, S, d, 1.0 / math.sqrt(d), bias=sp, out_dtype=torch.bfloat16)
        return _tail_bf16(x2d, hid, w["tail_self"]).view(B, S, C)

    def _forward_bf16(self, f, emb, w):
        B, S, C = f.shape[0] // 2, f.shape[1], f.shape[2]
        d = C // NUM_HEADS
        scale = 1.0 / math.sqrt(d)
        f = self._self_bf16(f, emb, w)
        out = torch.empty_like(f)
        x0, x1 = f[:B].view(B * S, C), f[B:].view(B * S, C)
        kq, vt_all = ops.gemm_tma_vt(f.view(2 * B * S, C), w["wkqv_c"].bf16, w["bkqv_c"], 2 * C, S, slot=1)
        kq1, vt1 = kq[B * S:], vt_all[B * C:]
        hid = ops.attn_tc(kq, C, kq1, 0, vt1, B, NUM_HEADS, S, S, d, scale, out_dtype=torch.bfloat16)
        _tail_bf16(x0, hid, w["tail_cross"], out=out[:B].view(B * S, C))
        k0, vt0 = ops.gemm_tma_vt(out[:B].view(B * S, C), w["wkv_c"].bf16, w["bkv_c"], C, S, slot=2)
        hid = ops.attn_tc(kq1, C, k0, 0, vt0, B, NUM_HEADS, S, S, d, scale, out_dtype=torch.bfloat16)
        _tail_bf16(x1, hid, w["tail_cross"], out=out[B:].view(B * S, C))
        return out

    @torch.no_grad()
    def forward(self, feats0, embeddings0, feats1, embeddings1, masks0=None, masks1=None):
        if masks0 is not None or masks1 is not None:
            raise NotImplementedError("key masks are never used on the SAM-6D inference path")
        w = self._weights()
        emb = _stack2(embeddings0, embeddings1) if feats0.shape == feats1.shape else None
        if emb is not None and self.precision == "bf16" and feats0.shape[1] <= 256:
            B = feats0.shape[0]
            f = _stack2(feats0, feats1)
            if f is None:
                f = torch.cat([feats0, feats1], dim=0)
            f = self._forward_bf16(f.to(torch.bfloat16).contiguous(), emb, w)
            return f[:B], f[B:]
        if emb is not None:
            B = feats0.shape[0]
            f = _stack2(feats0, feats1)
            f = self._self_layer(f if f is not None else torch.cat([feats0, feats1], dim=0), emb, w)
            feats0, feats1 = f[:B], f[B:]
        else:
            feats0 = self._self_layer(feats0.contiguous(), embeddings0, w)
            feats1 = self._self_layer(feats1.contiguous(), embeddings1, w)
        feats0 = self._cross_layer(feats0, feats1, w)
        feats1 = self._cross_layer(feats1, feats0, w)
        return feats0, feats1


class _SinusoidalBuffer(nn.Module):
    def __init__(self, d_model):
        super().__init__()
        div_indices = torch.arange(0, d_model, 2).float()
        self.register_buffer('div_term', torch.exp(div_indices * (-math.log(10000.0) / d_model)))


class GeometricStructureEmbedding(nn.Module):

    def __init__(self, cfg):
        super().__init__()
        cfg = _cfg(cfg)
        self.sigma_d, self.sigma_a, self.angle_k = cfg.sigma_d, cfg.sigma_a, cfg.angle_k
        self.factor_a = 180.0 / (self.sigma_a * math.pi)
        if cfg.reduction_a != 'max' or cfg.angle_k != 3 or cfg.hidden_dim != 256:
            raise ValueError("sam6d_b200 kernels are built for reduction_a='max', angle_k=3, hidden_dim=256")
        self.embedding = _SinusoidalBuffer(cfg.hidden_dim)
        self.proj_d = nn.Linear(cfg.hidden_dim, cfg.hidden_dim)
        self.proj_a = nn.Linear(cfg.hidden_dim, cfg.hidden_dim)
        self._packed = _Packed()
        self.precision = "fp32"

    def _weights(self):
        key = _param_key(self)
        if self._packed.key != key:
            self._packed.w = dict(div=_f32(self.embedding.div_term), waT=_f32(self.proj_a.weight).t().contiguous(),
                                  wdT=_f32(self.proj_d.weight).t().contiguous(),
                                  wd_bf=_f32(self.proj_d.weight).to(torch.bfloat16).contiguous(),
                                  bias=(_f32(self.proj_a.bias) + _f32(self.proj_d.bias)).contiguous())
            self._packed.w.update(self._tables(self._packed.w))
            self._packed.key = key
        return self._packed.w

    def _tables(self, w):
        div = w["div"].double()

        def table(weight, x_max, bias=None):
            n = int(math.ceil(x_max * GEO_LUT_INV_H)) + 1
            om = (torch.arange(n, dtype=torch.float64, device=div.device) / GEO_LUT_INV_H)[:, None] * div[None, :]
            emb = torch.stack([torch.sin(om), torch.cos(om)], dim=2).reshape(n, -1)
            g = emb @ weight.detach().double().t()
            if bias is not None:
                g = g + bias.double()
            return g.to(torch.float32).to(torch.bfloat16).contiguous()

        return dict(tab_a=table(self.proj_a.weight, 180.0 / self.sigma_a), tab_d=table(self.proj_d.weight, GEO_LUT_D_MAX, w["bias"]),
                    wdT_bf=_f32(self.proj_d.weight).t().contiguous().to(torch.bfloat16).contiguous())

    @torch.no_grad()
    def get_embedding_indices(self, points):
        T = ops.geo_indices(points.contiguous(), self.sigma_d, self.factor_a)
        return T[..., 3], T[..., :3]

    @torch.no_grad()
    def forward(self, points):
        w = self._weights()
        T = ops.geo_indices(points.contiguous(), self.sigma_d, self.factor_a)
        if self.precision == "bf16":
            far = ops.geo_embed_dist_tc(torch.stack([T[:, 0, :, :], T[:, :, 0, :]], dim=1).contiguous(), w["div"], w["wd_bf"], w["bias"])
            return ops.geo_embed_lut(T, w["tab_a"], GEO_LUT_INV_H, w["tab_d"], GEO_LUT_INV_H, far, w["div"], w["wdT_bf"], w["bias"])
        return ops.geo_embed_f32(T, w["div"], w["waT"], w["wdT"], w["bias"])


def sample_pts_feats(pts, feats, npoint=2048, return_index=False):
    idx = ops.furthest_point_sampling(pts.contiguous(), npoint)
    p = ops.gather_rows(pts.contiguous(), idx)
    f = ops.gather_rows_bf16_f32(feats.contiguous(), idx) if feats.dtype == torch.bfloat16 else ops.gather_rows(feats.contiguous(), idx)
    return (p, f, idx) if return_index else (p, f)


def compute_feature_similarity(feat1, feat2, type='cosine', temp=1.0, normalize_feat=True, precision="fp32"):
    if type != 'cosine':
        raise NotImplementedError("SAM-6D uses sim_type='cosine'")
    B, N, C = feat1.shape
    M = feat2.shape[1]
    ld = (M + 3) // 4 * 4
    store = torch.empty(B, N, ld, dtype=torch.float32, device=feat1.device)
    if precision == "bf16":
        f1 = ops.l2norm_rows_bf16(feat1.contiguous()) if normalize_feat else feat1.contiguous().to(torch.bfloat16)
        f2 = ops.l2norm_rows_bf16(feat2.contiguous()) if normalize_feat else feat2.contiguous().to(torch.bfloat16)
        ops.gemm_tma_batched(f1, f2, store, N, M, ld, N * ld, alpha=1.0 / temp)
    else:
        f1 = ops.l2norm_rows(feat1.contiguous()) if normalize_feat else feat1.contiguous()
        f2 = ops.l2norm_rows(feat2.contiguous()) if normalize_feat else feat2.contiguous()
        ops.gemm_raw(f1.data_ptr(), f2.data_ptr(), None, 0, store.data_ptr(), N, M, C, C, C, ld, 0, batch=B, sA=N * C, sW=M * C,
                     sC=N * ld, alpha=1.0 / temp)
    return store[:, :, :M]


def compute_coarse_Rt(atten, pts1, pts2, model_pts=None, n_proposal1=6000, n_proposal2=300, rand=None, return_scores=False):
    B = pts1.shape[0]
    if model_pts is None:
        model_pts = pts2
    W, w1 = ops.coarse_assign(atten.contiguous())
    if rand is None:
        rand = torch.rand(B, n_proposal1 * 3, device=pts1.device)
    idx = ops.coarse_sample(W, rand.contiguous())
    Rt, resid = ops.coarse_hypotheses(idx, pts1.contiguous(), pts2.contiguous())
    top = ops.topk_smallest(resid, n_proposal2)
    R, t, scores = ops.coarse_select(Rt, top, pts1.contiguous(), w1, model_pts.contiguous())
    if return_scores:
        return R, t, scores
    return R, t


def compute_fine_Rt(atten, pts1, pts2, model_pts=None, dis_thres=0.15, temp=0.1, radius=None, check_bound=True):
    if model_pts is None:
        model_pts = pts2
    bound = 1.0 / temp
    if check_bound and float(atten.abs().max()) > bound * (1.0 + 1e-3):
        raise ValueError(f"compute_fine_Rt: |atten| exceeds 1/temp = {bound:g}; the CUDA path handles cosine scores "
                         "(sim_type='cosine', normalize_feat=True) only")
    pts1, pts2 = pts1.contiguous(), pts2.contiguous()
    lab1, _, wts, pred = ops.fine_assign(atten, pts2, shift=1.0 / temp)
    R, t = ops.weighted_procrustes(pred, pts1, wts, 0.0, 1e-5)
    rad = radius if radius is not None else torch.ones(pts1.shape[0], device=pts1.device) - 1e-6
    score, t_scaled = ops.pose_score(pts1, lab1, R, t, model_pts.contiguous(), rad.contiguous(), dis_thres)
    return (R, t, score) if radius is None else (R, t, score, t_scaled)


class CoarsePointMatching(nn.Module):

    def __init__(self, cfg, return_feat=False):
        super().__init__()
        self.cfg = _cfg(cfg)
        self.return_feat = return_feat
        self.nblock = self.cfg.nblock
        self.in_proj = nn.Linear(self.cfg.input_dim, self.cfg.hidden_dim)
        self.out_proj = nn.Linear(self.cfg.hidden_dim, self.cfg.out_dim)
        self.bg_token = nn.Parameter(torch.randn(1, 1, self.cfg.hidden_dim) * .02)
        self.transformers = nn.ModuleList([
            GeometricTransformer(blocks=['self', 'cross'], d_model=self.cfg.hidden_dim, num_heads=4, dropout=None,
                                 activation_fn='ReLU', return_attention_scores=False) for _ in range(self.nblock)])
        self._packed = _Packed()
        self.precision = "fp32"

    def _weights(self):
        key = _param_key(self.in_proj) + _param_key(self.out_proj)
        if self._packed.key != key:
            self._packed.w = dict(w_in=_W(self.in_proj.weight), b_in=_f32(self.in_proj.bias), w_out=_W(self.out_proj.weight),
                                  b_out=_f32(self.out_proj.bias))
            self._packed.key = key
        return self._packed.w

    def _embed(self, f):
        B, n, C = f.shape
        w = self._weights()
        H = self.cfg.hidden_dim
        if self.precision == "bf16":
            out = torch.empty(B, n + 1, H, dtype=torch.bfloat16, device=f.device)
            out[:, 0, :] = self.bg_token.detach().reshape(1, -1).to(torch.bfloat16)
            ops.gemm_tc_raw(f.data_ptr(), 0, w["w_in"].bf16.data_ptr(), 1, w["b_in"], 0, out.data_ptr() + H * 2, 1, n, H, C, C, C, H, 0,
                            batch=B, sA=n * C, sW=0, sC=(n + 1) * H)
            return out
        out = torch.empty(B, n + 1, H, dtype=torch.float32, device=f.device)
        out[:, 0, :] = self.bg_token.detach().reshape(1, -1)
        _gemm_raw(self.precision, f.data_ptr(), w["w_in"], w["b_in"], 0, out.data_ptr() + H * 4, n, H, C, C, H, 0, batch=B,
                  sA=n * C, sC=(n + 1) * H)
        return out

    @torch.no_grad()
    def forward(self, p1, f1, geo1, p2, f2, geo2, radius, end_points, rand=None):
        if self.training:
            raise NotImplementedError("sam6d_b200 implements the inference path (model.eval())")
        f12 = _stack2(f1, f2)
        if f12 is not None:
            e = self._embed(f12)
            f1, f2 = e[:f1.shape[0]], e[f1.shape[0]:]
        else:
            f1 = self._embed(f1.contiguous())
            f2 = self._embed(f2.contiguous())
        for blk in self.transformers:
            f1, f2 = blk(f1, geo1, f2, geo2)
        B, S, H = f1.shape
        w = self._weights()
        f12 = _stack2(f1, f2)
        if f12 is not None:
            o = _gemm(self.precision, f12.reshape(2 * B * S, H), w["w_out"], w["b_out"]).view(2 * B, S, -1)
            o1, o2 = o[:B], o[B:]
        else:
            o1 = _gemm(self.precision, f1.reshape(B * S, H), w["w_out"], w["b_out"]).view(B, S, -1)
            o2 = _gemm(self.precision, f2.reshape(B * S, H), w["w_out"], w["b_out"]).view(B, S, -1)
        atten = compute_feature_similarity(o1, o2, self.cfg.sim_type, self.cfg.temp, self.cfg.normalize_feat, self.precision)
        model = ops.scale_by_radius(end_points['model'].contiguous(), radius.contiguous())
        init_R, init_t, self.last_select_scores = compute_coarse_Rt(atten, p1, p2, model, self.cfg.nproposal1,
                                                                    self.cfg.nproposal2, rand=rand, return_scores=True)
        end_points['init_R'] = init_R
        end_points['init_t'] = init_t
        if self.return_feat:
            return end_points, o1, o2
        return end_points


class _ConvBN(nn.Module):

    def __init__(self, cin, cout):
        super().__init__()
        self.conv = nn.Conv2d(cin, cout, kernel_size=(1, 1), bias=False)
        self.normlayer = nn.Module()
        self.normlayer.bn = nn.BatchNorm2d(cout)

    def folded(self):
        bn = self.normlayer.bn
        w = self.conv.weight.detach().double().reshape(self.conv.out_channels, -1)
        s = bn.weight.detach().double() / torch.sqrt(bn.running_var.detach().double() + bn.eps)
        return (w * s[:, None]).float().contiguous(), (bn.bias.detach().double() - bn.running_mean.detach().double() * s).float().contiguous()


class _SharedMLP(nn.Module):
    def __init__(self, dims):
        super().__init__()
        for i in range(len(dims) - 1):
            self.add_module(f"layer{i}", _ConvBN(dims[i], dims[i + 1]))


class _Conv1dParams(nn.Module):
    def __init__(self, cin, cout):
        super().__init__()
        self.conv = nn.Conv1d(cin, cout, kernel_size=1, bias=True)


class PositionalEncoding(nn.Module):

    def __init__(self, out_dim, r1=0.1, r2=0.2, nsample1=32, nsample2=64, use_xyz=True, bn=True):
        super().__init__()
        if not (use_xyz and bn) or (nsample1, nsample2) != (32, 64):
            raise ValueError("sam6d_b200 PositionalEncoding is built for the SAM-6D configuration")
        self.r1, self.r2, self.ns1, self.ns2 = r1, r2, nsample1, nsample2
        self.mlp1 = _SharedMLP([6, 32, 64, 128])
        self.mlp2 = _SharedMLP([6, 32, 64, 128])
        self.mlp3 = _Conv1dParams(256, out_dim)
        self._packed = _Packed()
        self.precision = "fp32"

    def _weights(self):
        key = _param_key(self)
        if self._packed.key != key:
            w = {}
            for name, mlp in (("m1", self.mlp1), ("m2", self.mlp2)):
                packed = []
                for j in range(3):
                    wj, bj = getattr(mlp, f"layer{j}").folded()
                    packed += [wj, bj]
                w[name] = tuple(packed)
                w[name + "_tc"] = (packed[0], packed[1], packed[2].to(torch.bfloat16).contiguous(), packed[3],
                                   packed[4].to(torch.bfloat16).contiguous(), packed[5])
            w["w3"] = _W(_f32(self.mlp3.conv.weight).reshape(self.mlp3.conv.out_channels, -1))
            w["b3"] = _f32(self.mlp3.conv.bias)
            self._packed.w, self._packed.key = w, key
        return self._packed.w

    @torch.no_grad()
    def local_features(self, pts):
        w = self._weights()
        pts = pts.contiguous()
        B, N, _ = pts.shape
        feat = torch.empty(B, N, 256, dtype=torch.bfloat16 if self.precision == "bf16" else torch.float32, device=pts.device)
        pair = ops.ball_query_pair(pts, pts, self.r1, self.ns1, self.r2, self.ns2) if self.r1 <= self.r2 else None
        for r, ns, name, off in ((self.r1, self.ns1, "m1", 0), (self.r2, self.ns2, "m2", 128)):
            if pair is not None:
                idx, cnt = pair[:2] if off == 0 else pair[2:]
            else:
                idx, cnt = ops.ball_query(pts, pts, r, ns, return_count=True)
            if self.precision == "bf16":
                ops.pe_mlp_max_tc(pts, idx, w[name + "_tc"], feat, off)
            else:
                ops.pe_mlp_max(pts, idx, cnt, w[name], feat, off)
        return feat

    @torch.no_grad()
    def forward(self, pts1, pts2=None):
        if pts2 is not None and pts2 is not pts1:
            raise NotImplementedError("SAM-6D always calls PE(pts) with a single cloud")
        w = self._weights()
        feat = self.local_features(pts1)
        B, N, _ = feat.shape
        if self.precision == "bf16":
            return ops.gemm_tma(feat.view(B * N, 256), w["w3"].bf16, w["b3"]).view(B, N, -1)
        return _gemm(self.precision, feat.view(B * N, 256), w["w3"], w["b3"]).view(B, N, -1)


class _LinearAttentionParams(nn.Module):
    def __init__(self, d_model):
        super().__init__()
        self.proj_q = nn.Linear(d_model, d_model)
        self.proj_k = nn.Linear(d_model, d_model)
        self.proj_v = nn.Linear(d_model, d_model)
        self.scale = nn.Parameter(torch.zeros(size=(1, 1, d_model)))


class _LinearAttentionLayerParams(nn.Module):
    def __init__(self, d_model):
        super().__init__()
        self.attention = _LinearAttentionParams(d_model)
        self.linear = nn.Linear(d_model, d_model)
        self.norm = nn.LayerNorm(d_model)


class _LinearTransformerLayerParams(nn.Module):
    def __init__(self, d_model):
        super().__init__()
        self.attention = _LinearAttentionLayerParams(d_model)
        self.output = _AttentionOutputParams(d_model)


class SparseToDenseTransformer(nn.Module):

    def __init__(self, d_model, sparse_blocks, num_heads=4, dropout=None, activation_fn='ReLU', parallel=False,
                 focusing_factor=3, with_bg_token=True, replace_bg_token=True):
        super().__init__()
        if not (with_bg_token and replace_bg_token) or focusing_factor != 3:
            raise ValueError("sam6d_b200 SparseToDenseTransformer is built for the SAM-6D configuration")
        self.d_model = d_model
        self.sparse_layer = GeometricTransformer(blocks=sparse_blocks, d_model=d_model, num_heads=num_heads, dropout=dropout,
                                                 activation_fn=activation_fn, parallel=parallel, return_attention_scores=False)
        self.dense_layer = _LinearTransformerLayerParams(d_model)
        self._packed = _Packed()
        self.precision = "fp32"

    def _weights(self):
        key = _param_key(self.dense_layer)
        if self._packed.key != key:
            la = self.dense_layer.attention.attention
            self._packed.w = dict(
                wq=_W(la.proj_q.weight), bq=_f32(la.proj_q.bias),
                wkv=_W(torch.cat([_f32(la.proj_k.weight), _f32(la.proj_v.weight)], dim=0)),
                bkv=torch.cat([_f32(la.proj_k.bias), _f32(la.proj_v.bias)], dim=0).contiguous(),
                sp_scale=torch.nn.functional.softplus(_f32(la.scale)).reshape(-1).contiguous(), tail=_pack_tail(self.dense_layer))
            self._packed.key = key
        return self._packed.w

    def _sample_feats(self, dense_feats, idx_ext):
        if dense_feats.dtype == torch.bfloat16:
            return ops.gather_rows_bf16(dense_feats, idx_ext)
        return ops.gather_rows(dense_feats, idx_ext)

    def _dense_layer_bf16(self, dense, sparse, w):
        B, N1, C = dense.shape
        N, J = N1 - 1, sparse.shape[1] - 1
        dev = dense.device
        bf = torch.bfloat16
        x2d = dense.view(B * N1, C)
        q = ops.gemm_tma(x2d, w["wq"].bf16, w["bq"], out_dtype=bf)
        kv = torch.empty(B * J, 2 * C, dtype=torch.float32, device=dev)
        s_bf = sparse.dtype == torch.bfloat16
        ops.gemm_tc_raw(sparse.data_ptr() + C * (2 if s_bf else 4), int(s_bf), w["wkv"].bf16.data_ptr(), 1, w["bkv"], 0, kv.data_ptr(), 0,
                        J, 2 * C, C, C, C, 2 * C, 0, batch=B, sA=(J + 1) * C, sW=0, sC=J * 2 * C)
        ops.focus_rows_raw(kv.data_ptr(), (B * J, 0, 2 * C), kv.data_ptr(), (B * J, 0, 2 * C), w["sp_scale"], B * J, C)
        blob, KS = ops.linattn_kv_pack_raw(kv.data_ptr(), 2 * C, J * 2 * C, kv.data_ptr() + C * 4, 2 * C, J * 2 * C, B, J, dev)
        x_att = torch.empty(B * N1, C, dtype=bf, device=dev)
        ops.linattn_tc_raw(q.data_ptr() + C * 2, C, N1 * C, blob, KS, w["sp_scale"], B, N, x_att.data_ptr() + C * 2, C, N1 * C)
        x_att.view(B, N1, C)[:, 0, :] = 0
        out = _tail_bf16(x2d, x_att, w["tail"]).view(B, N1, C)
        out[:, 0, :] = sparse[:, 0, :].to(bf)
        return out

    def _dense_layer(self, dense, sparse, w):
        B, N1, C = dense.shape
        N, J = N1 - 1, sparse.shape[1] - 1
        f = 4
        dev = dense.device
        x_ptr, x_view = dense.data_ptr() + C * f, (N, N1 * C, C)
        q = torch.empty(B * N, C, dtype=torch.float32, device=dev)
        prec = self.precision
        _gemm_raw(prec, x_ptr, w["wq"], w["bq"], 0, q.data_ptr(), N, C, C, C, C, 0, batch=B, sA=N1 * C, sC=N * C)
        kv = torch.empty(B * J, 2 * C, dtype=torch.float32, device=dev)
        _gemm_raw(prec, sparse.data_ptr() + C * f, w["wkv"], w["bkv"], 0, kv.data_ptr(), J, 2 * C, C, C, 2 * C, 0, batch=B,
                  sA=(J + 1) * C, sC=J * 2 * C)
        ops.focus_rows_raw(q.data_ptr(), (B * N, 0, C), q.data_ptr(), (B * N, 0, C), w["sp_scale"], B * N, C)
        ops.focus_rows_raw(kv.data_ptr(), (B * J, 0, 2 * C), kv.data_ptr(), (B * J, 0, 2 * C), w["sp_scale"], B * J, C)
        KV = torch.empty(B, NUM_HEADS, 64, 64, dtype=torch.float32, device=dev)
        KS = torch.empty(B, NUM_HEADS, 64, dtype=torch.float32, device=dev)
        ops.linattn_kv_raw(kv.data_ptr(), 2 * C, J * 2 * C, kv.data_ptr() + C * f, 2 * C, J * 2 * C, B, NUM_HEADS, J, KV, KS)
        x_att = torch.empty(B * N, C, dtype=torch.float32, device=dev)
        ops.linattn_apply_raw(q.data_ptr(), N, N * C, C, KV, KS, B, NUM_HEADS, x_att.data_ptr(), N * C, C)
        t = w["tail"]
        y = torch.empty(B * N, C, dtype=torch.float32, device=dev)
        _gemm_raw(prec, x_att.data_ptr(), t["wo"], t["bo"], x_ptr, y.data_ptr(), N, C, C, C, C, C, batch=B, sA=N * C, sC=N * C,
                  sR=N1 * C)
        y = ops.layernorm(y, t["g1"], t["b1"])
        h = _gemm(prec, y, t["we"], t["be"], relu=True)
        z = _gemm(prec, h, t["ws"], t["bs"], residual=y)
        out = torch.empty(B, N1, C, dtype=torch.float32, device=dev)
        ops.layernorm_raw(z.data_ptr(), (B * N, 0, C), out.data_ptr() + C * f, (N, N1 * C, C), t["g2"], t["b2"], B * N, C)
        out[:, 0, :] = sparse[:, 0, :]
        return out

    @torch.no_grad()
    def forward(self, dense_feats0, embeddings0, fps_idx0, dense_feats1, embeddings1, fps_idx1, masks0=None, masks1=None):
        w = self._weights()
        ext0 = torch.cat([torch.zeros_like(fps_idx0[:, :1]), fps_idx0], dim=1).contiguous()
        ext1 = torch.cat([torch.zeros_like(fps_idx1[:, :1]), fps_idx1], dim=1).contiguous()
        dense = _stack2(dense_feats0, dense_feats1)
        if dense is not None:
            B = dense_feats0.shape[0]
            feats = self._sample_feats(dense, torch.cat([ext0, ext1], dim=0))
            feats0, feats1 = self.sparse_layer(feats[:B], embeddings0, feats[B:], embeddings1, masks0, masks1)
            layer = self._dense_layer_bf16 if dense.dtype == torch.bfloat16 else self._dense_layer
            out = layer(dense, torch.cat([feats0, feats1], dim=0), w)
            return out[:B], out[B:]
        feats0 = self._sample_feats(dense_feats0.contiguous(), ext0)
        feats1 = self._sample_feats(dense_feats1.contiguous(), ext1)
        feats0, feats1 = self.sparse_layer(feats0, embeddings0, feats1, embeddings1, masks0, masks1)
        layer = self._dense_layer_bf16 if dense_feats0.dtype == torch.bfloat16 else self._dense_layer
        dense_feats0 = layer(dense_feats0.contiguous(), feats0, w)
        dense_feats1 = layer(dense_feats1.contiguous(), feats1, w)
        return dense_feats0, dense_feats1


class FinePointMatching(nn.Module):

    def __init__(self, cfg, return_feat=False):
        super().__init__()
        self.cfg = _cfg(cfg)
        self.return_feat = return_feat
        self.nblock = self.cfg.nblock
        self.in_proj = nn.Linear(self.cfg.input_dim, self.cfg.hidden_dim)
        self.out_proj = nn.Linear(self.cfg.hidden_dim, self.cfg.out_dim)
        self.bg_token = nn.Parameter(torch.randn(1, 1, self.cfg.hidden_dim) * .02)
        self.PE = PositionalEncoding(self.cfg.hidden_dim, r1=self.cfg.pe_radius1, r2=self.cfg.pe_radius2)
        self._packed = _Packed()
        self.precision = "fp32"
        self.transformers = nn.ModuleList([
            SparseToDenseTransformer(self.cfg.hidden_dim, num_heads=4, sparse_blocks=['self', 'cross'], dropout=None,
                                     activation_fn='ReLU', focusing_factor=self.cfg.focusing_factor, with_bg_token=True,
                                     replace_bg_token=True) for _ in range(self.nblock)])

    def _weights(self):
        key = _param_key(self.in_proj) + _param_key(self.out_proj)
        if self._packed.key != key:
            self._packed.w = dict(w_in=_W(self.in_proj.weight), b_in=_f32(self.in_proj.bias), w_out=_W(self.out_proj.weight),
                                  b_out=_f32(self.out_proj.bias))
            self._packed.key = key
        return self._packed.w

    def _embed(self, f, pts):
        B, N, C = f.shape
        H = self.cfg.hidden_dim
        w, pw = self._weights(), self.PE._weights()
        local = self.PE.local_features(pts)
        if self.precision == "bf16":
            f2d = f.reshape(B * N, C)
            if f2d.dtype == torch.bfloat16 and f2d.is_contiguous():
                tmp = ops.gemm_tma(f2d, w["w_in"].bf16, w["b_in"], out_dtype=torch.bfloat16)
            else:
                tmp = ops.gemm_tc(f2d, w["w_in"].bf16, w["b_in"], out_dtype=torch.bfloat16)
            out = torch.empty(B, N + 1, H, dtype=torch.bfloat16, device=f.device)
            out[:, 0, :] = self.bg_token.detach().reshape(1, -1).to(torch.bfloat16)
            ops.gemm_tma_batched(local, pw["w3"].bf16, out[:, 1:, :], N, H, H, (N + 1) * H, bias=pw["b3"],
                                 residual=tmp.view(B, N, H), ldr=H, r_bs=N * H)
            return out
        tmp = _gemm(self.precision, f.reshape(B * N, C), w["w_in"], w["b_in"])
        out = torch.empty(B, N + 1, H, dtype=torch.float32, device=f.device)
        out[:, 0, :] = self.bg_token.detach().reshape(1, -1)
        _gemm_raw(self.precision, local.data_ptr(), pw["w3"], pw["b3"], tmp.data_ptr(), out.data_ptr() + H * 4, N, H, 256, 256, H, H,
                  batch=B, sA=N * 256, sC=(N + 1) * H, sR=N * H)
        return out

    @torch.no_grad()
    def forward(self, p1, f1, geo1, fps_idx1, p2, f2, geo2, fps_idx2, radius, end_points):
        if self.training:
            raise NotImplementedError("sam6d_b200 implements the inference path (model.eval())")
        p1, p2 = p1.contiguous(), p2.contiguous()
        p1_ = ops.rigid_warp(p1, end_points['init_R'].contiguous(), end_points['init_t'].contiguous())
        f12 = _stack2(f1, f2) if p1.shape == p2.shape else None
        if f12 is not None:
            e = self._embed(f12, torch.cat([p1_, p2], dim=0))
            f1, f2 = e[:p1.shape[0]], e[p1.shape[0]:]
        else:
            f1 = self._embed(f1.contiguous(), p1_)
            f2 = self._embed(f2.contiguous(), p2)
        for blk in self.transformers:
            f1, f2 = blk(f1, geo1, fps_idx1, f2, geo2, fps_idx2)
        B, S, H = f1.shape
        w = self._weights()
        f12 = _stack2(f1, f2)
        if f12 is not None:
            o = _gemm(self.precision, f12.reshape(2 * B * S, H), w["w_out"], w["b_out"]).view(2 * B, S, -1)
            o1, o2 = o[:B], o[B:]
        else:
            o1 = _gemm(self.precision, f1.reshape(B * S, H), w["w_out"], w["b_out"]).view(B, S, -1)
            o2 = _gemm(self.precision, f2.reshape(B * S, H), w["w_out"], w["b_out"]).view(B, S, -1)
        model = ops.scale_by_radius(end_points['model'].contiguous(), radius.contiguous())
        if (self.precision == "bf16" and self.cfg.sim_type == 'cosine' and self.cfg.normalize_feat and H == 256
                and o1.shape[-1] == 256 and not self.return_feat):
            f1n, f2n = ops.l2norm_rows_bf16(o1.contiguous()), ops.l2norm_rows_bf16(o2.contiguous())
            lab1, _, wts, pred = ops.fine_assign_tc(f1n, f2n, p2, 1.0 / self.cfg.temp)
            pred_R, pred_t = ops.weighted_procrustes(pred, p1, wts, 0.0, 1e-5)
            score, t_scaled = ops.pose_score(p1, lab1, pred_R, pred_t, model.contiguous(), radius.contiguous(), 0.15)
        else:
            if not self.cfg.normalize_feat:
                raise NotImplementedError("FinePointMatching: normalize_feat=False scores are unbounded; the fixed-shift assignment "
                                          "kernels need cosine similarities (the SAM-6D configuration)")
            atten = compute_feature_similarity(o1, o2, self.cfg.sim_type, self.cfg.temp, self.cfg.normalize_feat, self.precision)
            pred_R, _, score, t_scaled = compute_fine_Rt(atten, p1, p2, model, temp=self.cfg.temp, radius=radius.contiguous(),
                                                         check_bound=False)
        end_points['pred_R'] = pred_R
        end_points['pred_t'] = t_scaled
        end_points['pred_pose_score'] = score
        if self.return_feat:
            return end_points, o1, o2
        return end_points


DEFAULT_MODEL_CFG = dict(
    coarse_npoint=196, fine_npoint=2048,
    geo_embedding=dict(sigma_d=0.2, sigma_a=15, angle_k=3, reduction_a='max', hidden_dim=256),
    coarse_point_matching=dict(nblock=3, input_dim=256, hidden_dim=256, out_dim=256, temp=0.1, sim_type='cosine',
                               normalize_feat=True, loss_dis_thres=0.15, nproposal1=6000, nproposal2=300),
    fine_point_matching=dict(nblock=3, input_dim=256, hidden_dim=256, out_dim=256, pe_radius1=0.1, pe_radius2=0.2,
                             focusing_factor=3, temp=0.1, sim_type='cosine', normalize_feat=True, loss_dis_thres=0.15),
)


class Net(nn.Module):

    def __init__(self, cfg=None, feature_extraction: Optional[nn.Module] = None, precision: str = "fp32"):
        super().__init__()
        cfg = _cfg(cfg if cfg is not None else DEFAULT_MODEL_CFG)
        self.cfg = cfg
        self.coarse_npoint = cfg.coarse_npoint
        self.fine_npoint = cfg.fine_npoint
        if feature_extraction is not None:
            self.feature_extraction = feature_extraction
        elif hasattr(cfg, "feature_extraction"):
            from .vit import ViTEncoder
            self.feature_extraction = ViTEncoder(cfg.feature_extraction, cfg.fine_npoint, precision)
        self.geo_embedding = GeometricStructureEmbedding(cfg.geo_embedding)
        self.coarse_point_matching = CoarsePointMatching(cfg.coarse_point_matching)
        self.fine_point_matching = FinePointMatching(cfg.fine_point_matching)
        self._graphs = None
        self.set_precision(precision)

    def enable_graphs(self, max_graphs: int = 8):
        from .graph import StepGraphs
        self._graphs = StepGraphs(max_graphs)
        return self

    def disable_graphs(self):
        self._graphs = None
        return self

    def set_precision(self, precision: str):
        if precision not in PRECISIONS:
            raise ValueError(f"precision must be one of {PRECISIONS}")
        self.precision = precision
        for m in self.modules():
            if hasattr(m, "precision") and m is not self:
                m.precision = precision
        return self

    def _features(self, end_points):
        if 'dense_fm' in end_points:
            dense_fm = end_points['dense_fm']
        elif hasattr(self, 'feature_extraction'):
            dense_fm = self.feature_extraction.get_img_feats(end_points['rgb'], end_points['rgb_choose'])
        else:
            raise RuntimeError("Net needs end_points['dense_fm'] or a feature_extraction module for the RGB branch")
        if 'dense_po' not in end_points or 'dense_fo' not in end_points:
            raise RuntimeError("inference needs the template bank: end_points['dense_po'], end_points['dense_fo']")
        dense_po = end_points['dense_po'].contiguous()
        radius = ops.cloud_radius(dense_po)
        dense_pm = ops.scale_by_radius(end_points['pts'].contiguous(), radius)
        dense_po = ops.scale_by_radius(dense_po, radius)
        return dense_pm, dense_fm.contiguous(), dense_po, end_points['dense_fo'].contiguous(), radius

    @torch.no_grad()
    def forward(self, end_points, rand=None, init_pose=None):
        if self.training:
            raise NotImplementedError("sam6d_b200 implements the inference path: call model.eval()")
        if self._graphs is not None and init_pose is None and 'pts' in end_points:
            n_rand = self.coarse_point_matching.cfg.nproposal1 * 3
            out = self._graphs.run(lambda ep, r: self._forward(ep, r, None), end_points, rand, n_rand,
                                   extra=(self.precision, hash(_param_key(self))))
            if out is not None:
                return out
        return self._forward(end_points, rand, init_pose)

    def _forward(self, end_points, rand, init_pose):
        dense_pm, dense_fm, dense_po, dense_fo, radius = self._features(end_points)
        B = dense_pm.size(0)
        if dense_pm.shape == dense_po.shape and dense_fm.shape == dense_fo.shape:
            pts2 = torch.cat([dense_pm, dense_po], dim=0)
            if self.precision == "bf16":
                fts2 = torch.empty(2 * B, *dense_fm.shape[1:], dtype=torch.bfloat16, device=dense_fm.device)
                fts2[:B].copy_(dense_fm)
                fts2[B:].copy_(dense_fo)
            else:
                fts2 = torch.cat([dense_fm, dense_fo], dim=0)
            dense_pm, dense_po, dense_fm, dense_fo = pts2[:B], pts2[B:], fts2[:B], fts2[B:]
            sp, sf, idx = sample_pts_feats(pts2, fts2, self.coarse_npoint, return_index=True)
            bg_point = torch.ones(2 * B, 1, 3, dtype=torch.float32, device=pts2.device) * 100
            geo = self.geo_embedding(torch.cat([bg_point, sp], dim=1))
            sparse_pm, sparse_po, sparse_fm, sparse_fo = sp[:B], sp[B:], sf[:B], sf[B:]
            fps_idx_m, fps_idx_o, geo_embedding_m, geo_embedding_o = idx[:B], idx[B:], geo[:B], geo[B:]
        else:
            bg_point = torch.ones(B, 1, 3, dtype=torch.float32, device=dense_pm.device) * 100
            sparse_pm, sparse_fm, fps_idx_m = sample_pts_feats(dense_pm, dense_fm, self.coarse_npoint, return_index=True)
            geo_embedding_m = self.geo_embedding(torch.cat([bg_point, sparse_pm], dim=1))
            sparse_po, sparse_fo, fps_idx_o = sample_pts_feats(dense_po, dense_fo, self.coarse_npoint, return_index=True)
            geo_embedding_o = self.geo_embedding(torch.cat([bg_point, sparse_po], dim=1))
        end_points = self.coarse_point_matching(sparse_pm, sparse_fm, geo_embedding_m, sparse_po, sparse_fo, geo_embedding_o,
                                                radius, end_points, rand=rand)
        if init_pose is not None:
            coarse_R, coarse_t = end_points['init_R'], end_points['init_t']
            end_points['init_R'], end_points['init_t'] = init_pose[0].contiguous(), init_pose[1].contiguous()
        end_points = self.fine_point_matching(dense_pm, dense_fm, geo_embedding_m, fps_idx_m, dense_po, dense_fo,
                                              geo_embedding_o, fps_idx_o, radius, end_points)
        if init_pose is not None:
            end_points['init_R'], end_points['init_t'] = coarse_R, coarse_t
        return end_points
```

Measured before the change: 2639.

## Fuse L2 norm into output GEMM and restructure fine-pass tensor-core pipeline

Adds an L2-normalize epilogue to the TMA GEMM so the output projection writes normalized bf16 features directly, which removes the separate l2norm kernels. The fine assignment kernel moves from BN=256 to BN=128 tiles with 8 stages. It double-buffers accumulators so reduction of one tile overlaps the wgmma of the next, and it handles a narrow remainder tile (S=2048+1 columns, 1 extra) with an N=8 wgmma instead of a full wide tile. The masked-points kernel is folded into mode 2 by loading lab2/pts2 inline, and per-warpgroup named barriers replace the CTA-wide one. This adds complexity and register pressure, and it risks ordering or pipeline-phase bugs.

New measurement: 2677 (median of 6 runs). +1.4%, better.

```diff
diff --git a/include/sam6d_b200.h b/include/sam6d_b200.h
--- a/include/sam6d_b200.h
+++ b/include/sam6d_b200.h
@@ -175,8 +175,8 @@
 int sam6d_fine_assign(const float* A, int B, int S, int ld, float shift, const float* pts2, float* rsum, float* csum, float* cpart,
                       int* cpi, int* lab1, int* lab2, float* wts, float* pred, void* stream);
 int sam6d_fine_pass_tc(const void* Fa, const void* Fb, int B, int S, float alpha, float shift, int mode, const float* row_f,
-                       const float* col_f, int ld_f, const float* q4, float* out_inv, int* lab, float* wts, float* pred, void* stream);
-int sam6d_fine_masked_points(const int* lab2, const float* pts2, int B, int S, int ld, float* q4, void* stream);
+                       const float* col_f, int ld_f, const int* lab2, const float* pts2, float* out_inv, int* lab, float* wts,
+                       float* pred, void* stream);
 int sam6d_weighted_procrustes(const float* src, const float* ref, const float* wts, int B, int N, float weight_thresh,
                               float eps, float* R, float* t, void* stream);
 int sam6d_pose_score(const float* pts1, const int* lab1, int B, int N, const float* R, const float* t, const float* model,
diff --git a/sam6d_b200/csrc/epilogue.cuh b/sam6d_b200/csrc/epilogue.cuh
--- a/sam6d_b200/csrc/epilogue.cuh
+++ b/sam6d_b200/csrc/epilogue.cuh
@@ -73,6 +73,31 @@
   }
 }
 
+__device__ __forceinline__ void store_frag_l2norm(float (&d)[128], int w, int lane, int row0, int M, float alpha,
+                                                  const float* __restrict__ bias, __nv_bfloat16* __restrict__ C, long long ldc) {
+  float ss[2] = {0.f, 0.f};
+#pragma unroll
+  for (int j = 0; j < 32; ++j) {
+    const int c = tc::frag_col(4 * j, lane);
+    const float b0 = __ldg(bias + c), b1 = __ldg(bias + c + 1);
+#pragma unroll
+    for (int h = 0; h < 2; ++h) {
+      const float x0 = fmaf(d[4 * j + 2 * h], alpha, b0), x1 = fmaf(d[4 * j + 2 * h + 1], alpha, b1);
+      d[4 * j + 2 * h] = x0; d[4 * j + 2 * h + 1] = x1;
+      ss[h] = fmaf(x1, x1, fmaf(x0, x0, ss[h]));
+    }
+  }
+  const float n[2] = {fmaxf(sqrtf(tc::quad_sum(ss[0])), 1e-12f), fmaxf(sqrtf(tc::quad_sum(ss[1])), 1e-12f)};
+#pragma unroll
+  for (int h = 0; h < 2; ++h) {
+    const int row = row0 + tc::frag_row(2 * h, w, lane);
+    if (row >= M) continue;
+#pragma unroll
+    for (int j = 0; j < 32; ++j)
+      st2(C + (size_t)row * ldc + tc::frag_col(4 * j, lane), d[4 * j + 2 * h] / n[h], d[4 * j + 2 * h + 1] / n[h]);
+  }
+}
+
 #define EPI_DISPATCH(ACT_V, BIAS_P, RES_P, ...)                                              \
   do {                                                                                       \
     const int a__ = (ACT_V);                                                                 \
diff --git a/sam6d_b200/csrc/fine_tc.cu b/sam6d_b200/csrc/fine_tc.cu
--- a/sam6d_b200/csrc/fine_tc.cu
+++ b/sam6d_b200/csrc/fine_tc.cu
@@ -1,11 +1,13 @@
+#include <type_traits>
+
 #include "common.cuh"
 #include "tc.cuh"
 
 namespace {
 
-constexpr int BM = 128, BN = 256, BK = 64, KB = 4, STAGES = 4;
-constexpr int A_KB = BM * BK * 2, B_KB = BN * BK * 2;
-constexpr int CONSUMERS = 256, NUM_THREADS = CONSUMERS + 128;
+constexpr int BM = 128, BN = 128, BT = 8, BK = 64, KB = 4, STAGES = 8;
+constexpr int A_KB = BM * BK * 2, B_KB = BN * BK * 2, T_KB = BT * BK * 2;
+constexpr int WG_THREADS = 128, CONSUMERS = 2 * WG_THREADS, NUM_THREADS = CONSUMERS + 128;
 constexpr int SMEM_BYTES = KB * A_KB + STAGES * B_KB + 1024;
 constexpr float LOG2E = 1.4426950408889634f;
 
@@ -14,31 +16,92 @@
   float a2, s2;
   const float* row_f;
   const float* col_f;
-  const float4* q4;
+  const int* lab2;
+  const float* pts2;
   float* out_inv;
   int* lab;
   float* wts; float* pred;
 };
 
+struct RowState {
+  float sum[2], bv[2], ws[2], px[2], py[2], pz[2];
+  int bi[2];
+};
+
+struct ColTiles {
+  int n_wide;
+  bool narrow;
+  __device__ explicit ColTiles(int S) {
+    const int r = S % BN;
+    narrow = r >= 1 && r <= BT;
+    n_wide = S / BN + ((r > BT) ? 1 : 0);
+  }
+};
+
+__device__ __forceinline__ void item_of(int q, int S, int B, int& b, int& mt) {
+  const int m_full = S / BM, n_full = B * m_full;
+  if (q < n_full) { b = q / m_full; mt = q - b * m_full; }
+  else { b = q - n_full; mt = m_full; }
+}
+
 __device__ __forceinline__ float ex2(float x) {
   float y;
   asm("ex2.approx.ftz.f32 %0, %1;" : "=f"(y) : "f"(x));
   return y;
 }
 
+template <int W>
+__device__ __forceinline__ void issue_tile(float (&acc)[W / 2], uint32_t a_addr, uint8_t* ring, uint64_t* full_bar, long long& gk) {
+#pragma unroll
+  for (int kb = 0; kb < KB; ++kb) {
+    const int s = (int)(gk % STAGES);
+    if (W == BN || kb == 0) tc::mbar_wait(&full_bar[s], (uint32_t)((gk / STAGES) & 1));
+    tc::wg_fence();
+    const uint32_t b_addr = tc::smem_u32(ring + s * B_KB) + (W == BN ? 0 : kb * T_KB);
+#pragma unroll
+    for (int k = 0; k < BK / 16; ++k)
+      tc::wgmma_bf16<W>(acc, tc::wg_desc(a_addr + kb * A_KB + k * 32), tc::wg_desc(b_addr + k * 32), (kb | k) ? 1u : 0u);
+    if (W == BN) ++gk;
+  }
+  if (W != BN) ++gk;
+  tc::wg_commit();
+}
+
+template <int MODE, int W>
+__device__ __forceinline__ void reduce_tile(const float (&acc)[W / 2], int lane, int col0, const FArgs& g, const float (&rf)[2],
+                                            const float* sc, const float4* sq, RowState& r) {
+#pragma unroll
+  for (int e = 0; e < W / 2; ++e) {
+    const int hr = (e >> 1) & 1, cl = tc::frag_col(e, lane), j = col0 + cl;
+    const float ev = (j < g.S) ? ex2(fmaf(acc[e], g.a2, -g.s2)) : 0.f;
+    if (MODE == 0) {
+      r.sum[hr] += ev;
+    } else {
+      const float p = (ev * rf[hr]) * (ev * sc[cl]);
+      if (p > r.bv[hr]) { r.bv[hr] = p; r.bi[hr] = j; }
+      if (MODE == 2) {
+        const float4 q = sq[cl];
+        const float pm = p * q.w;
+        r.ws[hr] += pm; r.px[hr] = fmaf(pm, q.x, r.px[hr]); r.py[hr] = fmaf(pm, q.y, r.py[hr]); r.pz[hr] = fmaf(pm, q.z, r.pz[hr]);
+      }
+    }
+  }
+}
+
 template <int MODE>
-__global__ void __launch_bounds__(NUM_THREADS, 1) fine_pass_kernel(const __grid_constant__ CUtensorMap tmA, const __grid_constant__ CUtensorMap tmB, FArgs g) {
+__global__ void __launch_bounds__(NUM_THREADS, 1) fine_pass_kernel(const __grid_constant__ CUtensorMap tmA, const __grid_constant__ CUtensorMap tmB,
+                                                                   const __grid_constant__ CUtensorMap tmT, FArgs g) {
   extern __shared__ __align__(1024) uint8_t smem_raw[];
   uint8_t* smem = reinterpret_cast<uint8_t*>((reinterpret_cast<uintptr_t>(smem_raw) + 1023) & ~(uintptr_t)1023);
   uint8_t* a_res = smem;
   uint8_t* ring = smem + KB * A_KB;
   __shared__ __align__(8) uint64_t a_full, a_empty, full_bar[STAGES], empty_bar[STAGES];
-  __shared__ float sc[2][BN];
-  __shared__ __align__(16) float4 sq[2][BN];
+  __shared__ float sc_all[2][2][BN];
+  __shared__ __align__(16) float4 sq_all[2][2][BN];
 
   const int tid = threadIdx.x, warp = tid >> 5, lane = tid & 31;
-  const int m_tiles = (g.S + BM - 1) / BM, n_tiles = (g.S + BN - 1) / BN;
-  const int items = g.B * m_tiles;
+  const ColTiles ct(g.S);
+  const int items = g.B * ((g.S + BM - 1) / BM);
 
   if (tid == 0) {
     tc::mbar_init(&a_full, 1); tc::mbar_init(&a_empty, CONSUMERS / 32);
@@ -46,6 +109,7 @@
     tc::mbar_fence_init();
     tc::tma_prefetch_desc(&tmA);
     tc::tma_prefetch_desc(&tmB);
+    tc::tma_prefetch_desc(&tmT);
   }
   __syncthreads();
 
@@ -54,102 +118,151 @@
     if (tid == CONSUMERS) {
       long long gk = 0;
       int it = 0;
-      for (int item = blockIdx.x; item < items; item += gridDim.x, ++it) {
-        const int b = item / m_tiles, mt = item - b * m_tiles;
+      for (int q = blockIdx.x; q < items; q += gridDim.x, ++it) {
+        int b, mt;
+        item_of(q, g.S, g.B, b, mt);
         tc::mbar_wait(&a_empty, (uint32_t)((it & 1) ^ 1));
         tc::mbar_arrive_expect_tx(&a_full, KB * A_KB);
         for (int kb = 0; kb < KB; ++kb) tc::tma_load_2d(&tmA, &a_full, a_res + kb * A_KB, kb * BK, b * g.S + mt * BM);
-        for (int nt = 0; nt < n_tiles; ++nt)
+        for (int nt = 0; nt < ct.n_wide; ++nt)
           for (int kb = 0; kb < KB; ++kb, ++gk) {
             const int s = (int)(gk % STAGES);
             tc::mbar_wait(&empty_bar[s], (uint32_t)(((gk / STAGES) & 1) ^ 1));
             tc::mbar_arrive_expect_tx(&full_bar[s], B_KB);
             tc::tma_load_2d(&tmB, &full_bar[s], ring + s * B_KB, kb * BK, b * g.S + nt * BN);
           }
+        if (ct.narrow) {
+          const int s = (int)(gk % STAGES);
+          tc::mbar_wait(&empty_bar[s], (uint32_t)(((gk / STAGES) & 1) ^ 1));
+          tc::mbar_arrive_expect_tx(&full_bar[s], KB * T_KB);
+          for (int kb = 0; kb < KB; ++kb) tc::tma_load_2d(&tmT, &full_bar[s], ring + s * B_KB + kb * T_KB, kb * BK, b * g.S + ct.n_wide * BN);
+          ++gk;
+        }
       }
     }
     return;
   }
   tc::consumer_regs();
-  const int wg = warp >> 2, w = warp & 3;
+  const int wg = __shfl_sync(0xffffffffu, warp >> 2, 0), w = warp & 3, wt = tid & (WG_THREADS - 1);
   const uint32_t a_addr = tc::smem_u32(a_res) + wg * (64 * 128);
-  long long gk = 0, tcount = 0;
+  float (*sc)[BN] = sc_all[wg];
+  float4 (*sq)[BN] = sq_all[wg];
+  long long gk = 0, gr = 0, tcount = 0;
   int it = 0;
-  for (int item = blockIdx.x; item < items; item += gridDim.x, ++it) {
-    const int b = item / m_tiles, mt = item - b * m_tiles;
+  for (int q = blockIdx.x; q < items; q += gridDim.x, ++it) {
+    int b, mt;
+    item_of(q, g.S, g.B, b, mt);
+    if (wg == 1 && g.S - mt * BM <= 64) {
+      const long long n_st = (long long)ct.n_wide * KB + (ct.narrow ? 1 : 0);
+      for (long long e = gk + n_st; gk < e; ++gk) {
+        tc::mbar_wait(&full_bar[gk % STAGES], (uint32_t)((gk / STAGES) & 1));
+        if (lane == 0) tc::mbar_arrive(&empty_bar[gk % STAGES]);
+      }
+      gr = gk;
+      if (lane == 0) tc::mbar_arrive(&a_empty);
+      continue;
+    }
+    const int i0 = mt * BM + wg * 64 + tc::frag_row(0, w, lane);
+    const bool rows = i0 < g.S;
     float rf[2] = {0.f, 0.f};
 #pragma unroll
+    for (int hr = 0; hr < 2; ++hr)
+      if (MODE != 0 && i0 + 8 * hr < g.S) rf[hr] = g.row_f[(size_t)b * g.ld_f + i0 + 8 * hr];
+    RowState r;
+#pragma unroll
     for (int hr = 0; hr < 2; ++hr) {
-      const int i = mt * BM + wg * 64 + tc::frag_row(2 * hr, w, lane);
-      if (MODE != 0 && i < g.S) rf[hr] = g.row_f[(size_t)b * g.ld_f + i];
-    }
-    const float* cf = (MODE != 0) ? g.col_f + (size_t)b * g.ld_f : nullptr;
-    const float4* q4 = (MODE == 2) ? g.q4 + (size_t)b * g.ld_f : nullptr;
-    float sum[2] = {0.f, 0.f}, bv[2] = {-INFINITY, -INFINITY}, ws[2] = {0.f, 0.f}, px[2] = {0.f, 0.f}, py[2] = {0.f, 0.f}, pz[2] = {0.f, 0.f};
-    int bi[2] = {0x7fffffff, 0x7fffffff};
+      r.sum[hr] = 0.f; r.bv[hr] = -INFINITY; r.ws[hr] = 0.f; r.px[hr] = 0.f; r.py[hr] = 0.f; r.pz[hr] = 0.f; r.bi[hr] = 0x7fffffff;
+    }
+    float st_c = 0.f;
+    float4 st_q = make_float4(0.f, 0.f, 0.f, 0.f);
+    auto stage_load = [&](int col0) {
+      if (MODE == 0) return;
+      const int j = col0 + wt;
+      st_c = (j < g.S) ? g.col_f[(size_t)b * g.ld_f + j] : 0.f;
+      if (MODE == 2) {
+        st_q = make_float4(0.f, 0.f, 0.f, 0.f);
+        if (j >= 1 && j < g.S) {
+          const float* p = g.pts2 + ((size_t)b * (g.S - 1) + (j - 1)) * 3;
+          const float x = p[0], y = p[1], z = p[2];
+          if (g.lab2[(size_t)b * g.S + j] > 0) st_q = make_float4(x, y, z, 1.f);
+        }
+      }
+    };
+    auto stage_store = [&](int buf) {
+      if (MODE == 0) return;
+      sc[buf][wt] = st_c;
+      if (MODE == 2) sq[buf][wt] = st_q;
+    };
+    stage_load(0);
+    stage_store((int)(tcount & 1));
     tc::mbar_wait(&a_full, (uint32_t)(it & 1));
-    for (int nt = 0; nt < n_tiles; ++nt, ++tcount) {
-      const int buf = (int)(tcount & 1);
+
+    float accA[BN / 2], accB[BN / 2];
+    auto finish = [&](float (&cur)[BN / 2], int nt, auto in_flight) {
+      const bool staged = nt + 1 < ct.n_wide || ct.narrow;
+      if (staged) stage_load((nt + 1) * BN);
+      tc::wg_wait<decltype(in_flight)::value>();
+      tc::acc_fence(cur);
+#pragma unroll
+      for (int kb = 0; kb < KB; ++kb, ++gr)
+        if (lane == 0) tc::mbar_arrive(&empty_bar[gr % STAGES]);
+      if (!staged && lane == 0) tc::mbar_arrive(&a_empty);
       if (MODE != 0) {
-        const int j = nt * BN + tid;
-        sc[buf][tid] = (j < g.S) ? cf[j] : 0.f;
-        if (MODE == 2) sq[buf][tid] = (j < g.S) ? q4[j] : make_float4(0.f, 0.f, 0.f, 0.f);
-        tc::named_bar(1, CONSUMERS);
-      }
-      float acc[BN / 2];
-      int prev = -1;
-      for (int kb = 0; kb < KB; ++kb, ++gk) {
-        const int s = (int)(gk % STAGES);
-        tc::mbar_wait(&full_bar[s], (uint32_t)((gk / STAGES) & 1));
-        const uint32_t b_addr = tc::smem_u32(ring + s * B_KB);
-        tc::wg_fence();
-#pragma unroll
-        for (int k = 0; k < BK / 16; ++k)
-          tc::wgmma_bf16<BN>(acc, tc::wg_desc(a_addr + kb * A_KB + k * 32), tc::wg_desc(b_addr + k * 32), (kb | k) ? 1u : 0u);
-        tc::wg_commit();
-        if (prev >= 0) {
-          tc::wg_wait<1>();
-          if (lane == 0) tc::mbar_arrive(&empty_bar[prev]);
-        }
-        prev = s;
-      }
+        tc::named_bar(1 + wg, WG_THREADS);
+        if (staged) stage_store((int)((tcount + 1) & 1));
+      }
+      if (rows) reduce_tile<MODE, BN>(cur, lane, nt * BN, g, rf, sc[tcount & 1], sq[tcount & 1], r);
+      ++tcount;
+    };
+    if (ct.n_wide > 0) {
+      const std::integral_constant<int, 0> none;
+      const std::integral_constant<int, 1> one;
+      int nt = 0;
+      issue_tile<BN>(accA, a_addr, ring, full_bar, gk);
+      for (; nt + 2 < ct.n_wide; nt += 2) {
+        issue_tile<BN>(accB, a_addr, ring, full_bar, gk);
+        finish(accA, nt, one);
+        issue_tile<BN>(accA, a_addr, ring, full_bar, gk);
+        finish(accB, nt + 1, one);
+      }
+      if (nt + 1 < ct.n_wide) {
+        issue_tile<BN>(accB, a_addr, ring, full_bar, gk);
+        finish(accA, nt, one);
+        finish(accB, nt + 1, none);
+      } else {
+        finish(accA, nt, none);
+      }
+    }
+    if (ct.narrow) {
+      float acc[BT / 2];
+      issue_tile<BT>(acc, a_addr, ring, full_bar, gk);
       tc::wg_wait<0>();
-      if (lane == 0) tc::mbar_arrive(&empty_bar[prev]);
-      if (nt == n_tiles - 1 && lane == 0) tc::mbar_arrive(&a_empty);
-#pragma unroll
-      for (int e = 0; e < BN / 2; ++e) {
-        const int hr = (e >> 1) & 1, cl = tc::frag_col(e, lane), j = nt * BN + cl;
-        const float ev = (j < g.S) ? ex2(fmaf(acc[e], g.a2, -g.s2)) : 0.f;
-        if (MODE == 0) {
-          sum[hr] += ev;
-        } else {
-          const float p = (ev * rf[hr]) * (ev * sc[buf][cl]);
-          if (p > bv[hr]) { bv[hr] = p; bi[hr] = j; }
-          if (MODE == 2) {
-            const float4 q = sq[buf][cl];
-            const float pm = p * q.w;
-            ws[hr] += pm; px[hr] = fmaf(pm, q.x, px[hr]); py[hr] = fmaf(pm, q.y, py[hr]); pz[hr] = fmaf(pm, q.z, pz[hr]);
-          }
-        }
-      }
+      tc::acc_fence(acc);
+      if (lane == 0) { tc::mbar_arrive(&empty_bar[gr % STAGES]); tc::mbar_arrive(&a_empty); }
+      ++gr;
+      if (MODE != 0) tc::named_bar(1 + wg, WG_THREADS);
+      if (rows) reduce_tile<MODE, BT>(acc, lane, ct.n_wide * BN, g, rf, sc[tcount & 1], sq[tcount & 1], r);
+      ++tcount;
     }
 #pragma unroll
     for (int hr = 0; hr < 2; ++hr) {
-      const int i = mt * BM + wg * 64 + tc::frag_row(2 * hr, w, lane);
+      const int i = i0 + 8 * hr;
       if (MODE == 0) {
-        const float t = tc::quad_sum(sum[hr]);
+        const float t = tc::quad_sum(r.sum[hr]);
         if ((lane & 3) == 0 && i < g.S) g.out_inv[(size_t)b * g.ld_f + i] = 1.f / t;
       } else {
+        float bv = r.bv[hr];
+        int bi = r.bi[hr];
 #pragma unroll
         for (int o = 1; o <= 2; o <<= 1) {
-          const float ov = __shfl_xor_sync(0xffffffffu, bv[hr], o);
-          const int oi = __shfl_xor_sync(0xffffffffu, bi[hr], o);
-          if (ov > bv[hr] || (ov == bv[hr] && oi < bi[hr])) { bv[hr] = ov; bi[hr] = oi; }
+          const float ov = __shfl_xor_sync(0xffffffffu, bv, o);
+          const int oi = __shfl_xor_sync(0xffffffffu, bi, o);
+          if (ov > bv || (ov == bv && oi < bi)) { bv = ov; bi = oi; }
         }
         float ww = 0.f, qx = 0.f, qy = 0.f, qz = 0.f;
-        if (MODE == 2) { ww = tc::quad_sum(ws[hr]); qx = tc::quad_sum(px[hr]); qy = tc::quad_sum(py[hr]); qz = tc::quad_sum(pz[hr]); }
+        if (MODE == 2) { ww = tc::quad_sum(r.ws[hr]); qx = tc::quad_sum(r.px[hr]); qy = tc::quad_sum(r.py[hr]); qz = tc::quad_sum(r.pz[hr]); }
         if ((lane & 3) == 0 && i < g.S) {
-          int lb = bi[hr];
+          int lb = bi;
           if (lb == 0x7fffffff) lb = 0;
           g.lab[(size_t)b * g.S + i] = lb;
           if (MODE == 2 && i >= 1) {
@@ -165,53 +278,35 @@
   }
 }
 
-__global__ void fine_masked_points_kernel(const int* __restrict__ lab2, const float* __restrict__ pts2, int S, int ld, float4* __restrict__ q4) {
-  const int b = blockIdx.y, j = blockIdx.x * blockDim.x + threadIdx.x;
-  if (j >= ld) return;
-  float4 q = make_float4(0.f, 0.f, 0.f, 0.f);
-  if (j >= 1 && j < S && lab2[(size_t)b * S + j] > 0) {
-    const float* p = pts2 + ((size_t)b * (S - 1) + (j - 1)) * 3;
-    q = make_float4(p[0], p[1], p[2], 1.f);
-  }
-  q4[(size_t)b * ld + j] = q;
-}
-
 }
 
 S6_API int sam6d_fine_pass_tc(const void* Fa, const void* Fb, int B, int S, float alpha, float shift, int mode, const float* row_f,
-                              const float* col_f, int ld_f, const float* q4, float* out_inv, int* lab, float* wts, float* pred,
-                              void* stream) {
+                              const float* col_f, int ld_f, const int* lab2, const float* pts2, float* out_inv, int* lab, float* wts,
+                              float* pred, void* stream) {
   S6_REQUIRE(Fa && Fb && B >= 0 && S >= 2 && mode >= 0 && mode <= 2 && ld_f >= S);
   S6_REQUIRE(((reinterpret_cast<uintptr_t>(Fa) | reinterpret_cast<uintptr_t>(Fb)) & 15) == 0 && (long long)B * S < 2000000000LL);
   if (mode == 0) S6_REQUIRE(out_inv != nullptr);
   if (mode >= 1) S6_REQUIRE(row_f && col_f && lab);
-  if (mode == 2) S6_REQUIRE(q4 && wts && pred && (reinterpret_cast<uintptr_t>(q4) & 15) == 0);
+  if (mode == 2) S6_REQUIRE(lab2 && pts2 && wts && pred);
   if (B == 0) return 0;
-  CUtensorMap tmA, tmB;
+  CUtensorMap tmA, tmB, tmT;
   int rc = tc::make_map_2d(&tmA, Fa, (long long)B * S, 256, 256, 64, BM);
   if (rc) return rc;
   rc = tc::make_map_2d(&tmB, Fb, (long long)B * S, 256, 256, 64, BN);
   if (rc) return rc;
+  rc = tc::make_map_2d(&tmT, Fb, (long long)B * S, 256, 256, 64, BT);
+  if (rc) return rc;
   int grid;
   S6_CHECK(s6_persistent_grid(B * s6_cdiv(S, BM), 1, &grid));
-  FArgs g{B, S, mode, ld_f, alpha * LOG2E, shift * LOG2E, row_f, col_f, reinterpret_cast<const float4*>(q4), out_inv, lab, wts, pred};
+  FArgs g{B, S, mode, ld_f, alpha * LOG2E, shift * LOG2E, row_f, col_f, lab2, pts2, out_inv, lab, wts, pred};
   cudaStream_t st = s6_stream(stream);
 #define FINE_LAUNCH(M)                                                                                              \
   do {                                                                                                              \
     S6_CHECK(cudaFuncSetAttribute(fine_pass_kernel<M>, cudaFuncAttributeMaxDynamicSharedMemorySize, SMEM_BYTES));   \
-    fine_pass_kernel<M><<<grid, NUM_THREADS, SMEM_BYTES, st>>>(tmA, tmB, g);                                        \
+    fine_pass_kernel<M><<<grid, NUM_THREADS, SMEM_BYTES, st>>>(tmA, tmB, tmT, g);                                   \
   } while (0)
   if (mode == 0) FINE_LAUNCH(0); else if (mode == 1) FINE_LAUNCH(1); else FINE_LAUNCH(2);
 #undef FINE_LAUNCH
   S6_LAUNCH_CHECK();
   return 0;
 }
-
-S6_API int sam6d_fine_masked_points(const int* lab2, const float* pts2, int B, int S, int ld, float* q4, void* stream) {
-  S6_REQUIRE(lab2 && pts2 && q4 && B >= 0 && S >= 2 && ld >= S && (reinterpret_cast<uintptr_t>(q4) & 15) == 0);
-  if (B == 0) return 0;
-  dim3 grid(s6_cdiv(ld, 256), B);
-  fine_masked_points_kernel<<<grid, 256, 0, s6_stream(stream)>>>(lab2, pts2, S, ld, reinterpret_cast<float4*>(q4));
-  S6_LAUNCH_CHECK();
-  return 0;
-}
diff --git a/sam6d_b200/csrc/gemm_tma.cu b/sam6d_b200/csrc/gemm_tma.cu
--- a/sam6d_b200/csrc/gemm_tma.cu
+++ b/sam6d_b200/csrc/gemm_tma.cu
@@ -117,6 +117,8 @@
       }
     } else if constexpr (ACT == 3) {
       epi::store_frag_swiglu(acc, w, lane, row0, g.M, n0, n0 / 2, g.alpha, g.bias, Cb, g.ldc);
+    } else if constexpr (ACT == 4) {
+      epi::store_frag_l2norm(acc, w, lane, row0, g.M, g.alpha, g.bias, Cb, g.ldc);
     } else {
       epi::store_frag<OT, ACT, HAS_BIAS, HAS_RES, OT, BN>(acc, w, lane, row0, g.M, n0, g.N, g.alpha, g.bias, Rb, g.ldr, Cb, g.ldc);
     }
@@ -127,7 +129,7 @@
                     long long lda, long long ldw, long long ldc, long long ldr, int batch, long long a_rpb, long long w_rpb,
                     long long c_bs, long long r_bs, float alpha, int act, void* stream, void* vt = nullptr, int vt_col0 = 0, int vt_S = 1,
                     int vt_N1 = 0, int vt_col1 = -1, void* c2 = nullptr, long long ldc2 = 0) {
-  S6_REQUIRE(A && W && C && M >= 0 && N > 0 && K > 0 && (K % 8) == 0 && (lda % 8) == 0 && (ldw % 8) == 0 && act >= 0 && act <= 3);
+  S6_REQUIRE(A && W && C && M >= 0 && N > 0 && K > 0 && (K % 8) == 0 && (lda % 8) == 0 && (ldw % 8) == 0 && act >= 0 && act <= 4);
   S6_REQUIRE((reinterpret_cast<uintptr_t>(A) & 15) == 0 && (reinterpret_cast<uintptr_t>(W) & 15) == 0 && batch >= 0);
   S6_REQUIRE(a_rpb * (long long)batch < 2000000000LL && w_rpb * (long long)batch < 2000000000LL);
   if (M == 0 || batch == 0) return 0;
@@ -169,6 +171,12 @@
     S6_LAUNCH_CHECK();
     return 0;
   }
+  if (act == 4) {
+    S6_REQUIRE(c_dtype == 1 && bias && !R && N == BN && (ldc % 2) == 0 && ldc >= N);
+    LAUNCH_ONE(__nv_bfloat16, 4, true, false, false);
+    S6_LAUNCH_CHECK();
+    return 0;
+  }
   EPI_DISPATCH(act, bias, R, LAUNCH_TMA);
 #undef LAUNCH_TMA
 #undef LAUNCH_ONE
diff --git a/sam6d_b200/csrc/tc.cuh b/sam6d_b200/csrc/tc.cuh
--- a/sam6d_b200/csrc/tc.cuh
+++ b/sam6d_b200/csrc/tc.cuh
@@ -86,6 +86,7 @@
                    : "l"(da), "l"(db), "r"(acc));                                                                            \
     }                                                                                                                        \
   };
+S6_WGMMA(8, "%0, %1, %2, %3", "%4", "%5", "%6", S6_F4(0))
 S6_WGMMA(16, S6_R0, "%8", "%9", "%10", S6_F8(0))
 S6_WGMMA(32, S6_R0 ", " S6_R1, "%16", "%17", "%18", S6_F16(0))
 S6_WGMMA(64, S6_R0 ", " S6_R1 ", " S6_R2 ", " S6_R3, "%32", "%33", "%34", S6_F32(0))
@@ -93,6 +94,12 @@
 S6_WGMMA(128, S6_R0 ", " S6_R1 ", " S6_R2 ", " S6_R3 ", " S6_R4 ", " S6_R5 ", " S6_R6 ", " S6_R7, "%64", "%65", "%66", S6_F64(0))
 S6_WGMMA(256, S6_R0 ", " S6_R1 ", " S6_R2 ", " S6_R3 ", " S6_R4 ", " S6_R5 ", " S6_R6 ", " S6_R7 ", " S6_R8 ", " S6_R9 ", " S6_R10
          ", " S6_R11 ", " S6_R12 ", " S6_R13 ", " S6_R14 ", " S6_R15, "%128", "%129", "%130", S6_F64(0), S6_F64(64))
+
+template <int N>
+__device__ __forceinline__ void acc_fence(float (&d)[N]) {
+#pragma unroll
+  for (int i = 0; i < N; ++i) asm volatile("" : "+f"(d[i])::"memory");
+}
 
 template <int N>
 __device__ __forceinline__ void wgmma_bf16(float (&d)[N / 2], uint64_t da, uint64_t db, uint32_t accumulate) {
diff --git a/sam6d_b200/ops.py b/sam6d_b200/ops.py
--- a/sam6d_b200/ops.py
+++ b/sam6d_b200/ops.py
@@ -172,7 +172,7 @@
         raise RuntimeError("gemm: inner dimensions differ")
     Nout = N // 2 if act == ACT_SWIGLU else N
     if out is None:
-        out = torch.empty(M, Nout, dtype=torch.bfloat16 if act == ACT_SWIGLU else out_dtype, device=A.device)
+        out = torch.empty(M, Nout, dtype=torch.bfloat16 if act in (ACT_SWIGLU, ACT_L2NORM) else out_dtype, device=A.device)
     if residual is not None:
         _check(residual, out.dtype, "residual", 2)
     _lib.call("sam6d_gemm_tma", _p(A), _p(W), _p(bias), _p(residual), _p(out), _DT[out.dtype], M, N, K, _ll(K), _ll(K), _ll(Nout), _ll(N),
@@ -181,6 +181,7 @@
 
 
 ACT_SWIGLU = 3
+ACT_L2NORM = 4
 
 
 def pack_swiglu_rows(t: Tensor, block: int = 128) -> Tensor:
@@ -699,18 +700,17 @@
     ld = (S + 3) // 4 * 4
     rinv = torch.empty(B, ld, dtype=torch.float32, device=dev)
     cinv = torch.empty(B, ld, dtype=torch.float32, device=dev)
-    q4 = torch.empty(B, ld, 4, dtype=torch.float32, device=dev)
     lab1 = torch.zeros(B, S, dtype=torch.int32, device=dev)
     lab2 = torch.zeros(B, S, dtype=torch.int32, device=dev)
     wts = torch.empty(B, S - 1, dtype=torch.float32, device=dev)
     pred = torch.empty(B, S - 1, 3, dtype=torch.float32, device=dev)
     a, sh = _f(alpha), _f(alpha)
-    _lib.call("sam6d_fine_pass_tc", _p(f1n), _p(f2n), B, S, a, sh, 0, None, None, ld, None, _p(rinv), None, None, None, _s())
-    _lib.call("sam6d_fine_pass_tc", _p(f2n), _p(f1n), B, S, a, sh, 0, None, None, ld, None, _p(cinv), None, None, None, _s())
-    _lib.call("sam6d_fine_pass_tc", _p(f2n), _p(f1n), B, S, a, sh, 1, _p(cinv), _p(rinv), ld, None, None, _p(lab2), None, None, _s())
-    _lib.call("sam6d_fine_masked_points", _p(lab2), _p(pts2), B, S, ld, _p(q4), _s())
-    _lib.call("sam6d_fine_pass_tc", _p(f1n), _p(f2n), B, S, a, sh, 2, _p(rinv), _p(cinv), ld, _p(q4), None, _p(lab1), _p(wts), _p(pred),
+    _lib.call("sam6d_fine_pass_tc", _p(f1n), _p(f2n), B, S, a, sh, 0, None, None, ld, None, None, _p(rinv), None, None, None, _s())
+    _lib.call("sam6d_fine_pass_tc", _p(f2n), _p(f1n), B, S, a, sh, 0, None, None, ld, None, None, _p(cinv), None, None, None, _s())
+    _lib.call("sam6d_fine_pass_tc", _p(f2n), _p(f1n), B, S, a, sh, 1, _p(cinv), _p(rinv), ld, None, None, None, _p(lab2), None, None,
               _s())
+    _lib.call("sam6d_fine_pass_tc", _p(f1n), _p(f2n), B, S, a, sh, 2, _p(rinv), _p(cinv), ld, _p(lab2), _p(pts2), None, _p(lab1),
+              _p(wts), _p(pred), _s())
     return lab1, lab2, wts, pred
 
 
diff --git a/sam6d_b200/pem.py b/sam6d_b200/pem.py
--- a/sam6d_b200/pem.py
+++ b/sam6d_b200/pem.py
@@ -737,21 +737,27 @@
             f1, f2 = blk(f1, geo1, fps_idx1, f2, geo2, fps_idx2)
         B, S, H = f1.shape
         w = self._weights()
-        f12 = _stack2(f1, f2)
-        if f12 is not None:
-            o = _gemm(self.precision, f12.reshape(2 * B * S, H), w["w_out"], w["b_out"]).view(2 * B, S, -1)
-            o1, o2 = o[:B], o[B:]
-        else:
-            o1 = _gemm(self.precision, f1.reshape(B * S, H), w["w_out"], w["b_out"]).view(B, S, -1)
-            o2 = _gemm(self.precision, f2.reshape(B * S, H), w["w_out"], w["b_out"]).view(B, S, -1)
         model = ops.scale_by_radius(end_points['model'].contiguous(), radius.contiguous())
         if (self.precision == "bf16" and self.cfg.sim_type == 'cosine' and self.cfg.normalize_feat and H == 256
-                and o1.shape[-1] == 256 and not self.return_feat):
-            f1n, f2n = ops.l2norm_rows_bf16(o1.contiguous()), ops.l2norm_rows_bf16(o2.contiguous())
+                and self.cfg.out_dim == 256 and not self.return_feat):
+            f12 = _stack2(f1, f2)
+            if f12 is not None:
+                o = ops.gemm_tma(f12.reshape(2 * B * S, H), w["w_out"].bf16, w["b_out"], act=ops.ACT_L2NORM).view(2 * B, S, -1)
+                f1n, f2n = o[:B], o[B:]
+            else:
+                f1n = ops.gemm_tma(f1.reshape(B * S, H), w["w_out"].bf16, w["b_out"], act=ops.ACT_L2NORM).view(B, S, -1)
+                f2n = ops.gemm_tma(f2.reshape(B * S, H), w["w_out"].bf16, w["b_out"], act=ops.ACT_L2NORM).view(B, S, -1)
             lab1, _, wts, pred = ops.fine_assign_tc(f1n, f2n, p2, 1.0 / self.cfg.temp)
             pred_R, pred_t = ops.weighted_procrustes(pred, p1, wts, 0.0, 1e-5)
             score, t_scaled = ops.pose_score(p1, lab1, pred_R, pred_t, model.contiguous(), radius.contiguous(), 0.15)
         else:
+            f12 = _stack2(f1, f2)
+            if f12 is not None:
+                o = _gemm(self.precision, f12.reshape(2 * B * S, H), w["w_out"], w["b_out"]).view(2 * B, S, -1)
+                o1, o2 = o[:B], o[B:]
+            else:
+                o1 = _gemm(self.precision, f1.reshape(B * S, H), w["w_out"], w["b_out"]).view(B, S, -1)
+                o2 = _gemm(self.precision, f2.reshape(B * S, H), w["w_out"], w["b_out"]).view(B, S, -1)
             if not self.cfg.normalize_feat:
                 raise NotImplementedError("FinePointMatching: normalize_feat=False scores are unbounded; the fixed-shift assignment "
                                           "kernels need cosine similarities (the SAM-6D configuration)")
```
